# zhihu/ZhiLight

Hardware: AMD Instinct MI355X
Metric: decode tokens/s (Llama-3-8B GPTQ-Int4, TP=1 per GPU, batch 1, seq 1024) (higher is better)
Workload: dtype f16; 1 GPU; Llama-3-8B GPTQ-Int4 g128 TP=1 batch=1 decode seq=1024 (BASELINE configs[1]); layers=32, parallelism=dp1 (independent TP=1 replicas), global_batch=1, seq_len=1024, valid=True, kv_cache_dtype=fp16, w4_algo=mfma

## Files before the change

### include/zhilight_amd.h

```cpp
#ifndef ZHILIGHT_AMD_H
#define ZHILIGHT_AMD_H

#include <stddef.h>
#include <stdint.h>

#ifdef __cplusplus
extern "C" {
#endif

#define ZL_VERSION 100

enum { ZL_F16 = 0, ZL_BF16 = 1, ZL_F32 = 2  };

enum {
    ZL_OK = 0,
    ZL_EINVAL = -1,
    ZL_ESHAPE = -2,
    ZL_EDTYPE = -3,
    ZL_ELIMIT = -4
};

typedef void* zl_stream_t;

int zl_version(void);
// ... 36 lines not shown

int zl_moe_grouped_bm(int64_t pairs, int64_t num_experts);
int64_t zl_moe_grouped_tiles(int64_t pairs, int64_t num_experts, int64_t bm);
int zl_w4a16_gemm_grouped(const uint16_t* x, int64_t ldx, int64_t x_rows, const uint32_t* qw, const uint32_t* meta,
                          int64_t num_experts, int64_t expert_stride_qw, int64_t expert_stride_meta,
                          const int32_t* expert_loads, const int32_t* index, int64_t pairs, int in_div, int out_scatter,
                          uint16_t* y, int64_t y_rows, int64_t n, int64_t k, int64_t group_size, int epilogue, zl_stream_t s);
int zl_w4a16_gemm_pairs(const uint16_t* x, int64_t ldx, int64_t x_rows, const uint32_t* qw, const uint32_t* meta, int64_t num_experts,
                        int64_t expert_stride_qw, int64_t expert_stride_meta, const int32_t* expert_ids, int64_t pairs, int in_div,
                        uint16_t* y, int64_t n, int64_t k, int64_t group_size, int epilogue, zl_stream_t s);

enum {
    ZL_EPI_BIAS = 1, ZL_EPI_ADD_C = 2, ZL_EPI_RESIDUAL = 4, ZL_EPI_SILU_MUL = 8, ZL_EPI_SILU_MUL_F32 = 16
};

int zl_w4a16_gemm(const uint16_t* x, int64_t ldx,
                  const uint32_t* qw, const uint16_t* scales, const uint16_t* zeros,
                  const uint16_t* bias, const uint16_t* residual, uint16_t* y,
                  int64_t m, int64_t n, int64_t k, int64_t group_size, int sym,
                  const uint16_t* norm_weight, float norm_eps, int epilogue, zl_stream_t s);

int zl_w4m_layout(int64_t n, int64_t k, int64_t group_size, zl_w4_layout_t* out);
int zl_w4m_pack(const uint32_t* qweight_km, const uint8_t* qzeros_km, const uint16_t* scales_km,
                int64_t n, int64_t k, int64_t group_size, int row_interleave,
                uint32_t* qw, uint32_t* meta, zl_stream_t s);
int zl_w4m_unpack(const uint32_t* qw, const uint32_t* meta, int64_t n, int64_t k, int64_t group_size, int row_interleave,
                  uint32_t* qweight_km, uint8_t* qzeros_km, uint16_t* scales_km, zl_stream_t s);
int zl_w4a16_gemm_mfma(const uint16_t* x, int64_t ldx,
                       const uint32_t* qw, const uint32_t* meta,
                       const uint16_t* bias, const uint16_t* residual, uint16_t* y,
                       int64_t m, int64_t n, int64_t k, int64_t group_size,
                       const uint16_t* norm_weight, float norm_eps, int epilogue, zl_stream_t s);

#define ZL_SCRATCH_HEADER 65536
typedef struct {
    void* scratch;
    int64_t scratch_bytes;
    int phase_rounds, phase_ksplit, phase_ksplit_min_m, phase_min_m, phase_max_m, phase_small_off;
    int tiled_min_m, tiled_bm, tiled_splitk;
    int mfma_ks, mfma_rounds;
    int small_algo;
    int tiled_wide;
    int slab;
    int slab_min_m;
    int slab_nw, slab_gpw;
    int slab_r;
    int defer_norm;
    const float* row_ss;
    float* row_ss_out;
} zl_w4_opts_t;
int64_t zl_w4a16_scratch_bytes(int64_t m, int64_t n);
int zl_row_ss(const uint16_t* x, int64_t ldx, int64_t m, int64_t k, float* out, zl_stream_t s);
int zl_w4a16_emits_row_ss(int64_t m, int64_t n, int64_t k, int64_t group_size, int epilogue, const zl_w4_opts_t* opts);
int zl_w4a16_takes_row_ss(int64_t m, int64_t n, int64_t k, int64_t group_size, int rope, const zl_w4_opts_t* opts);
int zl_w4a16_gemm_mfma_ex(const uint16_t* x, int64_t ldx, const uint32_t* qw, const uint32_t* meta, const uint16_t* bias,
                          const uint16_t* residual, uint16_t* y, int64_t m, int64_t n, int64_t k, int64_t group_size,
                          const uint16_t* norm_weight, float norm_eps, int epilogue, const zl_w4_opts_t* opts, zl_stream_t s);
int zl_w4a16_gemm_tiled(const uint16_t* x, int64_t ldx, const uint32_t* qw, const uint32_t* meta,
                        const uint16_t* bias, const uint16_t* residual, uint16_t* y,
                        int64_t m, int64_t n, int64_t k, int64_t group_size, int epilogue, zl_stream_t s);
int zl_w4a16_gemm_tiled_ex(const uint16_t* x, int64_t ldx, const uint32_t* qw, const uint32_t* meta,
                           const uint16_t* bias, const uint16_t* residual, uint16_t* y, int64_t m, int64_t n, int64_t k,
                           int64_t group_size, int epilogue, const zl_w4_opts_t* opts, zl_stream_t s);


int zl_gemm_nt_small_m(const uint16_t* x, int64_t ldx, const uint16_t* w , const uint16_t* bias,
                       uint16_t* y, int64_t m, int64_t n, int64_t k, float alpha, int dtype,
                       const uint16_t* norm_weight, float norm_eps, zl_stream_t s);
int zl_gemm_nt(const uint16_t* x, int64_t ldx, const uint16_t* w , const uint16_t* bias, uint16_t* y,
               int64_t m, int64_t n, int64_t k, float alpha, int dtype, zl_stream_t s);
int64_t zl_dense_m_bytes(int64_t n, int64_t k);
int zl_dense_pack_m(const uint16_t* w, uint16_t* out, int64_t n, int64_t k, zl_stream_t s);
int zl_gemm_nt_packed(const uint16_t* x, int64_t ldx, const uint16_t* wp, const uint16_t* bias, uint16_t* y, int64_t m,
                      int64_t n, int64_t k, float alpha, int dtype, zl_stream_t s);
int zl_gemm_nt_f32(const uint16_t* x, int64_t ldx, const uint16_t* w , float* y, int64_t m, int64_t n, int64_t k, float alpha,
                   int dtype, zl_stream_t s);

int64_t zl_argmax_workspace_bytes(int64_t m, int64_t n);
int zl_gemm_nt_small_m_argmax(const uint16_t* x, int64_t ldx, const uint16_t* w , const uint16_t* bias,
                              uint16_t* y, int64_t m, int64_t n, int64_t k, float alpha, int dtype,
                              const uint16_t* norm_weight, float norm_eps, void* argmax_ws, zl_stream_t s);
int zl_greedy_advance(const void* argmax_ws, int64_t m, int64_t n, int32_t* tokens, int32_t* positions,
                      int32_t* placement, int32_t* valid_lens, int64_t* next_tokens, zl_stream_t s);

int64_t zl_lm_head_score_ws_bytes(int64_t m, int64_t n);
int zl_lm_head_score(const uint16_t* x, int64_t ldx, const uint16_t* w , const int32_t* labels, int32_t ignore_index,
                     int32_t col0, float* lse, float* label_logit, float* logprob, int32_t* greedy, float* greedy_logit,
                     void* workspace, int64_t m, int64_t n, int64_t k, int dtype, zl_stream_t s);
enum { ZL_SCORE_ORDER_AUTO = -1 };
int zl_lm_head_score_ex(const uint16_t* x, int64_t ldx, const uint16_t* w , const int32_t* labels, int32_t ignore_index,
                        int32_t col0, float* lse, float* label_logit, float* logprob, int32_t* greedy, float* greedy_logit,
                        void* workspace, int64_t m, int64_t n, int64_t k, int dtype, int order, zl_stream_t s);


int zl_fp8_calc_scale(const uint16_t* x, int64_t numel, float max_e4m3, float* scale, int dtype, zl_stream_t s);
int zl_fp8_cvt_half(const uint16_t* x, const float* scale, uint8_t* out, int64_t numel, int dtype, zl_stream_t s);
int zl_fp8_gemm_nt(const uint8_t* a , const uint8_t* b , const float* scale_a, const float* scale_b,
                   uint16_t* out , int64_t m, int64_t n, int64_t k, zl_stream_t s);

int zl_quant_group_32(const uint16_t* x, int8_t* q, uint16_t* scale, int64_t groups, int dtype, zl_stream_t s);
int zl_dequant_sum_quant_g32(const uint16_t* my , const int8_t* q_others ,
                             const uint16_t* scale_others , int8_t* q_sum, uint16_t* scale_sum,
                             int64_t groups, int world_size, int dtype, zl_stream_t s);
int zl_dequant_group_32(const int8_t* q, const uint16_t* scale, uint16_t* out, int64_t groups, int dtype, zl_stream_t s);

int zl_rmsnorm(const uint16_t* x, const uint16_t* weight, uint16_t* out, int64_t rows, int64_t dim,
               float eps, float scale, const uint16_t* x2, uint16_t* out_sum, int dtype, zl_stream_t s);

int zl_rope_cos_sin(const int32_t* pos, float* cosv, float* sinv, int64_t s_len, int64_t d, float base,
                    int neox, zl_stream_t s);
int zl_rope_cos_sin_llama3(const int32_t* pos, float* cosv, float* sinv, int64_t s_len, int64_t d, float base,
                           float factor, float low_freq_factor, float high_freq_factor,
                           float old_context_len, int neox, zl_stream_t s);
int zl_rope_cos_sin_dynamic(const int32_t* pos, const int32_t* seq_len, float* cosv, float* sinv, int64_t s_len, int64_t d,
                            float base, float factor, float max_position_embeddings, int neox, zl_stream_t s);
int zl_rope_cos_sin_yarn(const int32_t* pos, float* cosv, float* sinv, int64_t s_len, int64_t d, float base, float factor,
                         float low, float high, float mscale, int neox, zl_stream_t s);
int zl_head_norm(const uint16_t* x, const uint16_t* weight, uint16_t* out, int64_t rows, int64_t heads, int64_t d, int64_t ld_in,
                 int64_t ld_out, float eps, int mode, int dtype, zl_stream_t s);
int zl_rotary_embedding_qk(const int32_t* pos, const uint16_t* in, uint16_t* q, uint16_t* k, uint16_t* v,
                           int64_t s_len, int64_t h, int64_t hkv, int64_t d, float theta, int dtype,
                           zl_stream_t s);
int zl_rope_qk_cache(const float* cosv, const float* sinv, const uint16_t* in, uint16_t* q, uint16_t* k,
                     uint16_t* v, int64_t s_len, int64_t h, int64_t hkv, int64_t d, int neox, int dtype,
                     zl_stream_t s);
int zl_rope_rotate(const float* cosv, const float* sinv, const uint16_t* x, uint16_t* out, int64_t n, int64_t heads, int64_t d,
                   int64_t x_stride_n, int64_t x_stride_h, int64_t out_stride_n, int64_t out_stride_h, int neox, int dtype, zl_stream_t s);
int zl_mask_valid_lens(const int8_t* mask, const int32_t* buf_lens, int32_t* valid_lens, int64_t b, int64_t len_q, zl_stream_t s);

int zl_copy_to_rag_buffer2(const int32_t* placement, const int32_t* buf_lens, const uint16_t* k_src,
                           const uint16_t* v_src, uint16_t* const* k_bufs, uint16_t* const* v_bufs,
                           int64_t b, int64_t len_q, int64_t hkv, int64_t d, int bshd, zl_stream_t s);
int zl_copy_to_rag_buffer_bytes(const int32_t* placement, const int32_t* buf_lens, const void* k_src, const void* v_src, void* const* k_bufs,
                                void* const* v_bufs, int64_t b, int64_t len_q, int64_t hkv, int64_t row_bytes, int bshd, zl_stream_t s);
int zl_kv_blocks_copy(const int32_t* desc, int64_t n, void* const* k_bufs, void* const* v_bufs, const int32_t* buf_lens, void* pool,
                      int64_t layers, int64_t b, int64_t block, int64_t hkv, int64_t row_bytes, int bshd, int to_pool, zl_stream_t s);
int zl_kv_blocks_copy_ex(const int32_t* desc, int64_t n, void* const* k_bufs, void* const* v_bufs, const int32_t* buf_lens, void* pool,
                         int64_t layers, int64_t b, int64_t block, int64_t hkv, int64_t row_bytes, int bshd, int to_pool,
                         int64_t piece_bytes, zl_stream_t s);

int zl_rope_scatter_decode(const float* cosv, const float* sinv, const uint16_t* qkv ,
                           uint16_t* q , const int32_t* placement ,
                           const int32_t* buf_lens, uint16_t* const* k_bufs, uint16_t* const* v_bufs,
                           int64_t b, int64_t h, int64_t hkv, int64_t d, int neox, int bshd, int dtype,
                           zl_stream_t s);

int64_t zl_decode_attn_workspace_bytes(int64_t b, int64_t len_q, int64_t h, int64_t d, int64_t max_len_buf);
int zl_decode_attn(const uint16_t* q, const int32_t* buf_lens, const uint16_t* const* k_bufs,
                   const uint16_t* const* v_bufs, const int8_t* mask, const int32_t* valid_lens,
                   uint16_t* out, void* workspace, int64_t b, int64_t len_q, int64_t h, int64_t hkv,
                   int64_t d, float scale, int64_t max_len_buf, int bshd, int dtype, zl_stream_t s);
int zl_decode_attn_ex(const uint16_t* q, const int32_t* buf_lens, const uint16_t* const* k_bufs,
                      const uint16_t* const* v_bufs, const int8_t* mask, const int32_t* valid_lens,
                      uint16_t* out, void* workspace, int64_t b, int64_t len_q, int64_t h, int64_t hkv,
                      int64_t d, float scale, int64_t max_len_buf, int bshd, int dtype, int algo, zl_stream_t s);

int zl_decode_attn_causal(const uint16_t* q, const int32_t* buf_lens, const uint16_t* const* k_bufs,
                          const uint16_t* const* v_bufs, const int32_t* valid_lens, uint16_t* out, void* workspace,
                          int64_t b, int64_t len_q, int64_t h, int64_t hkv, int64_t d, float scale, int64_t max_len_buf,
                          int bshd, int dtype, zl_stream_t s);

int zl_decode_attn_fused(const float* cosv, const float* sinv, const uint16_t* qkv, const int32_t* placement,
                         const int32_t* buf_lens, const int32_t* valid_lens, uint16_t* const* k_bufs,
                         uint16_t* const* v_bufs, uint16_t* out, void* workspace, int64_t b, int64_t h,
                         int64_t hkv, int64_t d, float scale, int64_t max_len_buf, int neox, int bshd, int dtype,
                         zl_stream_t s);
// ... 320 lines not shown
```

### zhilight_amd/_lib.py

```python
import ctypes as C
import os

import torch

_HERE = os.path.dirname(os.path.abspath(__file__))
SO_PATH = os.environ.get("ZHILIGHT_AMD_SO") or os.path.join(_HERE, "libzhilight_amd.so")

SYMBOLS = [
    "zl_mla_decode_workspace_bytes", "zl_mla_decode_attn", "zl_mla_decode_attn_ex", "zl_mla_decode_attn_paged",
    "zl_moe_sum_experts", "zl_moe_sum_experts_arr", "zl_moe_route_shared_lb", "zl_moe_plus_for_sort", "zl_moe_calc_reverse_idx",
    "zl_moe_fill_m_indices",
    "zl_embedding_rope",
    "zl_fp8_per_token_cast", "zl_fp8_block_dequant", "zl_fp8_block_gemm_group", "zl_fp8_block_packed_bytes", "zl_fp8_block_pack", "zl_fp8_block_gemm_group_packed", "zl_moe_top_k_softmax", "zl_moe_group_topk",
    "zl_cast", "zl_copy_2d", "zl_index_select", "zl_argmax_advance", "zl_arange_i32", "zl_divide_i32", "zl_scatter_update_dim0", "zl_sort_pairs_i32", "zl_log_softmax_bias", "zl_softmax_rows", "zl_topk_rows", "zl_gather_logits", "zl_scatter_logits", "zl_repetition_penalty", "zl_spec_accept", "zl_lookup_draft", "zl_stop_advance", "zl_slots_admit", "zl_sample_advance", "zl_spec_sample_accept", "zl_sample_advance_ex", "zl_spec_sample_accept_ex", "zl_seen_mark", "zl_sample_advance_opts", "zl_spec_sample_accept_opts", "zl_sample_advance_fsm", "zl_spec_sample_accept_fsm", "zl_slots_admit_fsm", "zl_reduce_abs_max", "zl_binary_op", "zl_scale", "zl_act_inplace",
    "zl_count_nonfinite", "zl_perm_narrow_u16", "zl_perm_reverse_u16", "zl_permute_input_u16", "zl_gptq_permute_rows",
    "zl_version", "zl_status_string", "zl_device_cu_count",
    "zl_gptq_shuffle", "zl_gptq_increase_zero", "zl_gptq_q4_to_q8", "zl_transpose_2d", "zl_gptq_reconstruct",
    "zl_awq_un_shuffle", "zl_awq_shuffle",
    "zl_w4_layout", "zl_w4_pack", "zl_w4_dequant", "zl_w4a16_gemm",
    "zl_w4m_layout", "zl_w4m_pack", "zl_w4m_unpack", "zl_w4a16_gemm_mfma", "zl_w4a16_gemm_tiled", "zl_w4a16_scratch_bytes", "zl_w4a16_gemm_mfma_ex", "zl_w4a16_gemm_tiled_ex",
    "zl_gemm_nt_small_m", "zl_gemm_nt", "zl_gemm_nt_f32", "zl_argmax_workspace_bytes", "zl_gemm_nt_small_m_argmax", "zl_greedy_advance",
    "zl_lm_head_score_ws_bytes", "zl_lm_head_score", "zl_lm_head_score_ex",
    "zl_rmsnorm",
    "zl_w4a16_moe_up", "zl_w4a16_moe_down", "zl_moe_grouped_bm", "zl_moe_grouped_tiles", "zl_w4a16_gemm_grouped", "zl_w4a16_gemm_pairs", "zl_rope_cos_sin", "zl_rope_cos_sin_llama3", "zl_rope_cos_sin_dynamic", "zl_rope_cos_sin_yarn", "zl_head_norm", "zl_rotary_embedding_qk", "zl_rope_qk_cache", "zl_rope_rotate", "zl_mask_valid_lens",
    "zl_copy_to_rag_buffer2", "zl_copy_to_rag_buffer_bytes", "zl_kv_blocks_copy", "zl_kv_blocks_copy_ex", "zl_rope_scatter_decode", "zl_w4a16_qkv_rope_scatter", "zl_w4a16_qkv_rope_scatter_ex", "zl_decode_attn_splits_h", "zl_decode_attn_splits_h_mask", "zl_decode_attn_combine_h", "zl_w4a16_gemm_attn_merge_h", "zl_w4a16_gemm_attn_merge_h_ex",
    "zl_quant_group_32", "zl_dequant_sum_quant_g32", "zl_dequant_group_32",
    "zl_fp8_calc_scale", "zl_fp8_cvt_half", "zl_fp8_gemm_nt",
    "zl_decode_attn_workspace_bytes", "zl_decode_attn", "zl_decode_attn_ex", "zl_decode_attn_causal", "zl_decode_attn_fused",
    "zl_decode_attn_split_len", "zl_decode_attn_splits", "zl_w4a16_gemm_attn_merge",
    "zl_decode_attn_la_split_len", "zl_decode_attn_la_workspace_bytes", "zl_decode_attn_la",
    "zl_quant_calc_scale_zp", "zl_dequant_group", "zl_quant_copy_to_rag_buffer", "zl_rope_quant_scatter_decode", "zl_decode_attn_quant", "zl_decode_attn_quant_ex",
    "zl_prefill_attn", "zl_prefill_attn_ex", "zl_prefill_attn_varlen", "zl_prefill_attn_varlen_q8",
    "zl_element_add_scale", "zl_gate_mul", "zl_gate_fuse", "zl_dense_m_bytes", "zl_dense_pack_m", "zl_gemm_nt_packed", "zl_row_ss", "zl_w4a16_emits_row_ss", "zl_w4a16_takes_row_ss", "zl_permute_input", "zl_embedding",
    "zl_w8m_bytes", "zl_w8m_pack", "zl_w8a8_gemm_phase", "zl_w8a8_gemm_phase_ex", "zl_w8a8_qkv_rope_scatter",
    "zl_quant_calc_scale", "zl_rmsnorm_quant", "zl_int8_gemm_nt", "zl_quant_scale_back",
    "zl_quant_back_act_mul", "zl_quant_scale_back3", "zl_quant_back_element_add_scale", "zl_quant_back_transpose",
    "zl_quant_back_copy_to_buffer",
    "zl_w4a8_weight_to_int8", "zl_quant_scale_back_f32",
    "zl_awq_dequantize", "zl_awq_gemm_workspace_bytes", "zl_awq_gemm",
]


EXPERIMENTAL_SYMBOLS = ["zl_w4a16_attn_out_gate_up", "zl_engine_epoch_advance",
                        "zl_w4a16_planes_bytes", "zl_w4a16_planes", "zl_w4a16_gemm_planes", "zl_w4a16_qkv_rope_scatter_planes"]
experimental = False


class W4Opts(C.Structure):
    _fields_ = [("scratch", C.c_void_p), ("scratch_bytes", C.c_int64)] + [(n, C.c_int) for n in (
        "phase_rounds", "phase_ksplit", "phase_ksplit_min_m", "phase_min_m", "phase_max_m", "phase_small_off",
        "tiled_min_m", "tiled_bm", "tiled_splitk", "mfma_ks", "mfma_rounds", "small_algo", "tiled_wide",
        "slab", "slab_min_m", "slab_nw", "slab_gpw", "slab_r", "defer_norm")] + [("row_ss", C.c_void_p), ("row_ss_out", C.c_void_p)]


class W4Layout(C.Structure):
    _fields_ = [(n, C.c_int64) for n in
                ("n", "k", "group_size", "np", "kp", "q", "c", "qw_bytes", "scales_bytes", "zeros_bytes")]


_lib = None


def lib():
    global _lib
    if _lib is None:
        if not os.path.exists(SO_PATH):
            raise ImportError(
                f"{SO_PATH} not found: build it with `python -m zhilight_amd.build` "
                "(hipcc --offload-arch=gfx950). zhilight_amd has no CPU/PyTorch fallback.")
        l = C.CDLL(SO_PATH)
        for name in SYMBOLS:
            getattr(l, name)
        l.zl_status_string.restype = C.c_char_p
        l.zl_decode_attn_workspace_bytes.restype = C.c_int64
        l.zl_decode_attn_split_len.restype = C.c_int64
        l.zl_decode_attn_la_split_len.restype = C.c_int64
        l.zl_decode_attn_la_workspace_bytes.restype = C.c_int64
        l.zl_argmax_workspace_bytes.restype = C.c_int64
        l.zl_lm_head_score_ws_bytes.restype = C.c_int64
        l.zl_w8m_bytes.restype = C.c_int64
        l.zl_dense_m_bytes.restype = C.c_int64
        l.zl_fp8_block_packed_bytes.restype = C.c_int64
        l.zl_mla_decode_workspace_bytes.restype = C.c_int64
        l.zl_w4a16_scratch_bytes.restype = C.c_int64
        l.zl_moe_grouped_tiles.restype = C.c_int64
        global experimental
        experimental = all(hasattr(l, name) for name in EXPERIMENTAL_SYMBOLS)
        if experimental:
            l.zl_w4a16_planes_bytes.restype = C.c_int64
        l.zl_awq_gemm_workspace_bytes.restype = C.c_int64
        l.zl_sample_advance.restype = C.c_int
        l.zl_sample_advance.argtypes = [C.c_void_p, C.c_int] + [C.c_int64] * 3 + [C.c_void_p] * 14
        l.zl_spec_sample_accept.restype = C.c_int
        l.zl_spec_sample_accept.argtypes = [C.c_void_p, C.c_int] + [C.c_int64] * 4 + [C.c_void_p] * 17
        l.zl_sample_advance_ex.restype = C.c_int
        l.zl_sample_advance_ex.argtypes = [C.c_void_p, C.c_int] + [C.c_int64] * 3 + [C.c_void_p] * 16 + [C.c_int64, C.c_void_p]
        l.zl_spec_sample_accept_ex.restype = C.c_int
        l.zl_spec_sample_accept_ex.argtypes = [C.c_void_p, C.c_int] + [C.c_int64] * 4 + [C.c_void_p] * 19 + [C.c_int64, C.c_void_p]
        opts = [C.c_void_p] * 3 + [C.c_int64, C.c_void_p, C.c_int64, C.c_int, C.c_void_p, C.c_void_p]
        l.zl_sample_advance_opts.restype = C.c_int
        l.zl_sample_advance_opts.argtypes = [C.c_void_p, C.c_int] + [C.c_int64] * 3 + [C.c_void_p] * 16 + [C.c_int64] + opts + [C.c_void_p]
        l.zl_spec_sample_accept_opts.restype = C.c_int
        l.zl_spec_sample_accept_opts.argtypes = [C.c_void_p, C.c_int] + [C.c_int64] * 4 + [C.c_void_p] * 19 + [C.c_int64] + opts + [C.c_void_p]
        fsm = [C.c_void_p, C.c_int64] + [C.c_void_p] * 4 + [C.c_int64] * 2 + [C.c_void_p]
# ... 56 lines not shown
```

### zhilight_amd/csrc/dense_gemv.hip

```cpp
#include "zl_common.h"
#include "zl_stage.h"

namespace {

constexpr int kRing = 8;

struct DenseParams {
    const uint16_t* x;
    int64_t ldx;
    const uint16_t* w;
    const uint16_t* bias;
    uint16_t* y;
    const uint16_t* norm_w;
    float norm_eps, alpha;
    int m, n, k, kp;
    int loads_per_row;
    int rows_per_wave;
    float2* argmax_ws;
    int total_waves;
};

typedef _Float16 hv2 __attribute__((ext_vector_type(2)));

template <int DT>
__device__ __forceinline__ float dot8(uint4 a, uint4 b, float acc) {
    const uint32_t au[4] = {a.x, a.y, a.z, a.w}, bu[4] = {b.x, b.y, b.z, b.w};
#pragma unroll
    for (int e = 0; e < 4; ++e) {
        if constexpr (DT == ZL_F16) {
            acc = __builtin_amdgcn_fdot2(__builtin_bit_cast(hv2, au[e]), __builtin_bit_cast(hv2, bu[e]), acc, false);
        } else {
            acc = __builtin_fmaf(__builtin_bit_cast(float, au[e] << 16), __builtin_bit_cast(float, bu[e] << 16), acc);
            acc = __builtin_fmaf(__builtin_bit_cast(float, au[e] & 0xffff0000u),
                                 __builtin_bit_cast(float, bu[e] & 0xffff0000u), acc);
        }
    }
    return acc;
}

template <int DT, int MT>
__global__ __launch_bounds__(256) void k_dense_gemv(const DenseParams p) {
    extern __shared__ __attribute__((aligned(16))) unsigned char smem[];
    uint16_t* xs = reinterpret_cast<uint16_t*>(smem);
    float* red = reinterpret_cast<float*>(smem + (size_t)MT * p.kp * 2);

    const int lane = threadIdx.x & 63;
    const int wave = __builtin_amdgcn_readfirstlane(threadIdx.x >> 6);
    const int m0 = blockIdx.y * MT;
    const int L = p.loads_per_row;
    const int gw = blockIdx.x * 4 + wave;
    const int row0 = gw * p.rows_per_wave;
    int nrows = p.n - row0;
    nrows = nrows < 0 ? 0 : (nrows > p.rows_per_wave ? p.rows_per_wave : nrows);
    const int total = nrows * L;

    uint4 wq[kRing];
    int iss_row = row0, iss_l = 0;
    auto issue = [&](int slot) {
        const int col = iss_l * 512 + lane * 8;
        uint4 v = make_uint4(0, 0, 0, 0);
        if (col < p.k) v = zl_load_nt(reinterpret_cast<const uint4*>(p.w + (size_t)iss_row * p.k + col));
        wq[slot] = v;
        if (++iss_l == L) {
            iss_l = 0;
            ++iss_row;
        }
    };
#pragma unroll
    for (int s = 0; s < kRing; ++s)
        if (s < total) issue(s);

    zl_stage_rows<DT, MT, 256>(p.x, p.ldx, m0, p.m, p.k, p.kp, p.norm_w, p.norm_eps, xs, red);
    __syncthreads();

    float acc[MT];
    float best_v[MT];
    int best_i[MT];
#pragma unroll
    for (int m = 0; m < MT; ++m) {
        acc[m] = 0.f;
        best_v[m] = -INFINITY;
        best_i[m] = 0x7fffffff;
    }
    int cl = 0, crow = row0;
    auto consume = [&](int slot) {
#pragma unroll
        for (int m = 0; m < MT; ++m) {
            uint4 xa = *reinterpret_cast<const uint4*>(xs + (size_t)m * p.kp + cl * 512 + lane * 8);
            acc[m] = dot8<DT>(wq[slot], xa, acc[m]);
        }
        if (++cl == L) {
            cl = 0;
#pragma unroll
            for (int m = 0; m < MT; ++m) {
                float v = zl_wave_sum(acc[m]);
                acc[m] = 0.f;
                if (lane == 0 && (m0 + m) < p.m) {
                    float b = p.bias ? ZT<DT>::to_f32(p.bias[crow]) : 0.f;
                    const uint16_t y16 = ZT<DT>::from_f32(p.alpha * v + b);
                    p.y[(size_t)(m0 + m) * p.n + crow] = y16;
                    const float yv = ZT<DT>::to_f32(y16);
                    if (yv > best_v[m] || best_i[m] == 0x7fffffff || (yv != yv && best_v[m] == best_v[m])) {
                        best_v[m] = yv;
                        best_i[m] = crow;
                    }
                }
            }
            ++crow;
        }
    };
#pragma unroll 1
    for (int it = 0; it < total; it += kRing) {
#pragma unroll
        for (int s = 0; s < kRing; ++s) {
            if (it + s < total) {
                consume(s);
                if (it + s + kRing < total) issue(s);
            }
        }
    }
    if (p.argmax_ws && lane == 0) {
#pragma unroll
        for (int m = 0; m < MT; ++m)
            if ((m0 + m) < p.m)
                p.argmax_ws[(size_t)(m0 + m) * p.total_waves + gw] = make_float2(best_v[m], __int_as_float(best_i[m]));
    }
}

__device__ __forceinline__ bool greedy_beats(float v, int i, float bv, int bi) {
    if (i == 0x7fffffff) return false;
    if (bi == 0x7fffffff) return true;
    if (v != v) return bv == bv || i < bi;
    return v > bv || (v == bv && i < bi);
}

__global__ __launch_bounds__(256) void k_greedy_advance(const float2* ws, int total_waves, int32_t* tokens,
                                                        int32_t* positions, int32_t* placement, int32_t* valid_lens,
                                                        int64_t* next_out) {
    __shared__ float sv[256];
    __shared__ int si[256];
    const int b = blockIdx.x;
    float bv = -INFINITY;
    int bi = 0x7fffffff;
    for (int w0 = threadIdx.x; w0 < total_waves; w0 += 4 * 256) {
        float2 c[4];
#pragma unroll
        for (int u = 0; u < 4; ++u) {
            const int w = w0 + u * 256;
            c[u] = w < total_waves ? ws[(size_t)b * total_waves + w] : make_float2(0.f, __int_as_float(0x7fffffff));
        }
#pragma unroll
        for (int u = 0; u < 4; ++u) {
            const int ci = __float_as_int(c[u].y);
            if (greedy_beats(c[u].x, ci, bv, bi)) {
                bv = c[u].x;
                bi = ci;
            }
        }
    }
    sv[threadIdx.x] = bv;
    si[threadIdx.x] = bi;
    __syncthreads();
    for (int off = 128; off > 0; off >>= 1) {
        if ((int)threadIdx.x < off) {
            const float ov = sv[threadIdx.x + off];
            const int oi = si[threadIdx.x + off];
            if (greedy_beats(ov, oi, sv[threadIdx.x], si[threadIdx.x])) {
                sv[threadIdx.x] = ov;
                si[threadIdx.x] = oi;
            }
        }
        __syncthreads();
    }
    if (threadIdx.x == 0) {
        const int tok = si[0] == 0x7fffffff ? 0 : si[0];
        if (tokens) tokens[b] = tok;
        if (next_out) next_out[b] = tok;
        if (positions) positions[b] += 1;
        if (placement) placement[b] += 1;
        if (valid_lens) valid_lens[b] += 1;
    }
}

template <int DT, int MT>
int launch(const DenseParams& p, int gx, int gy, hipStream_t st) {
    size_t lds = (size_t)MT * p.kp * 2 + 64;
    if (lds > 160 * 1024) return ZL_ELIMIT;
    if (lds > 64 * 1024) {
        hipError_t e = hipFuncSetAttribute(reinterpret_cast<const void*>(&k_dense_gemv<DT, MT>),
                                           hipFuncAttributeMaxDynamicSharedMemorySize, (int)lds);
        if (e != hipSuccess) return (int)e;
    }
    hipLaunchKernelGGL((k_dense_gemv<DT, MT>), dim3(gx, gy), dim3(256), lds, st, p);
    return zl_launch_status();
}

template <int DT>
__global__ __launch_bounds__(64) void k_gemm_nt_f32(const uint16_t* __restrict__ x, int64_t ldx, const uint16_t* __restrict__ w, float* __restrict__ y,
                                                    int n, int k, float alpha) {
    const int col = blockIdx.x, row = blockIdx.y, lane = threadIdx.x;
    const uint16_t* xr = x + (int64_t)row * ldx;
    const uint16_t* wr = w + (int64_t)col * k;
    float acc = 0.f;
    for (int i = lane * 8; i + 8 <= k; i += 64 * 8) {
        const uint4 a = *reinterpret_cast<const uint4*>(xr + i), b = *reinterpret_cast<const uint4*>(wr + i);
        const uint32_t au[4] = {a.x, a.y, a.z, a.w}, bu[4] = {b.x, b.y, b.z, b.w};
#pragma unroll
        for (int e = 0; e < 4; ++e) {
            acc = __builtin_fmaf(ZT<DT>::to_f32((uint16_t)(au[e] & 0xffffu)), ZT<DT>::to_f32((uint16_t)(bu[e] & 0xffffu)), acc);
            acc = __builtin_fmaf(ZT<DT>::to_f32((uint16_t)(au[e] >> 16)), ZT<DT>::to_f32((uint16_t)(bu[e] >> 16)), acc);
        }
    }
    acc = zl_wave_sum(acc);
    if (lane == 0) y[(int64_t)row * n + col] = alpha * acc;
}

}

static int dense_waves(int64_t n, int* rows_per_wave, int* gx) {
    int cus = zl_device_cu_count();
    if (cus <= 0) cus = 256;
    const int waves = cus * 8;
    *rows_per_wave = (int)((n + waves - 1) / waves);
    *gx = (int)(((n + *rows_per_wave - 1) / *rows_per_wave + 3) / 4);
    return *gx * 4;
}

extern "C" int64_t zl_argmax_workspace_bytes(int64_t m, int64_t n) {
    if (m <= 0 || n <= 0) return ZL_EINVAL;
    int rpw, gx;
    return m * (int64_t)dense_waves(n, &rpw, &gx) * 8;
}

static int gemm_nt_small_m_impl(const uint16_t* x, int64_t ldx, const uint16_t* w, const uint16_t* bias, uint16_t* y,
                                int64_t m, int64_t n, int64_t k, float alpha, int dtype, const uint16_t* norm_weight,
                                float norm_eps, void* argmax_ws, zl_stream_t s) {
    ZL_CHECK_ARG(x && w && y && m > 0 && n > 0 && k > 0, ZL_EINVAL);
    ZL_CHECK_ARG(k % 8 == 0 && ldx % 8 == 0 && ldx >= k, ZL_ESHAPE);
    ZL_CHECK_ARG(dtype == ZL_F16 || dtype == ZL_BF16, ZL_EDTYPE);
    DenseParams p;
    p.x = x; p.ldx = ldx; p.w = w; p.bias = bias; p.y = y;
    p.norm_w = norm_weight; p.norm_eps = norm_eps; p.alpha = alpha;
    p.m = (int)m; p.n = (int)n; p.k = (int)k;
    p.kp = (int)((k + 511) / 512 * 512);
    p.loads_per_row = p.kp / 512;
    int mt = m >= 4 ? 4 : (int)m;
    while (mt > 1 && (size_t)mt * p.kp * 2 + 64 > 64 * 1024) --mt;
    if (mt == 3) mt = 2;
    const int gy = (int)((m + mt - 1) / mt);
    int gx;
    p.total_waves = dense_waves(n, &p.rows_per_wave, &gx);
    p.argmax_ws = reinterpret_cast<float2*>(argmax_ws);
    hipStream_t hs = (hipStream_t)s;
#define ZL_DISPATCH(DT)                                      \
    switch (mt) {                                            \
        case 1: return launch<DT, 1>(p, gx, gy, hs);         \
        case 2: return launch<DT, 2>(p, gx, gy, hs);         \
        default: return launch<DT, 4>(p, gx, gy, hs);        \
    }
    if (dtype == ZL_F16) { ZL_DISPATCH(ZL_F16) }
    ZL_DISPATCH(ZL_BF16)
#undef ZL_DISPATCH
}

extern "C" int zl_gemm_nt_small_m(const uint16_t* x, int64_t ldx, const uint16_t* w, const uint16_t* bias, uint16_t* y,
                                  int64_t m, int64_t n, int64_t k, float alpha, int dtype,
                                  const uint16_t* norm_weight, float norm_eps, zl_stream_t s) {
    return gemm_nt_small_m_impl(x, ldx, w, bias, y, m, n, k, alpha, dtype, norm_weight, norm_eps, nullptr, s);
}

extern "C" int zl_gemm_nt_small_m_argmax(const uint16_t* x, int64_t ldx, const uint16_t* w, const uint16_t* bias,
                                         uint16_t* y, int64_t m, int64_t n, int64_t k, float alpha, int dtype,
                                         const uint16_t* norm_weight, float norm_eps, void* argmax_ws, zl_stream_t s) {
    ZL_CHECK_ARG(argmax_ws, ZL_EINVAL);
    return gemm_nt_small_m_impl(x, ldx, w, bias, y, m, n, k, alpha, dtype, norm_weight, norm_eps, argmax_ws, s);
}

extern "C" int zl_gemm_nt_f32(const uint16_t* x, int64_t ldx, const uint16_t* w, float* y, int64_t m, int64_t n, int64_t k, float alpha, int dtype,
                              zl_stream_t s) {
    ZL_CHECK_ARG(x && w && y && m > 0 && n > 0 && k > 0, ZL_EINVAL);
    ZL_CHECK_ARG(k % 8 == 0 && ldx >= k && ldx % 8 == 0 && ((uintptr_t)x & 15) == 0 && ((uintptr_t)w & 15) == 0 && m <= 65535 && n < ((int64_t)1 << 31), ZL_ESHAPE);
    ZL_CHECK_ARG(dtype == ZL_F16 || dtype == ZL_BF16, ZL_EDTYPE);
    const dim3 grid((unsigned)n, (unsigned)m);
    if (dtype == ZL_F16) hipLaunchKernelGGL(k_gemm_nt_f32<ZL_F16>, grid, dim3(64), 0, (hipStream_t)s, x, ldx, w, y, (int)n, (int)k, alpha);
    else hipLaunchKernelGGL(k_gemm_nt_f32<ZL_BF16>, grid, dim3(64), 0, (hipStream_t)s, x, ldx, w, y, (int)n, (int)k, alpha);
    return zl_launch_status();
}

extern "C" int zl_greedy_advance(const void* argmax_ws, int64_t m, int64_t n, int32_t* tokens, int32_t* positions,
                                 int32_t* placement, int32_t* valid_lens, int64_t* next_tokens, zl_stream_t s) {
    ZL_CHECK_ARG(argmax_ws && m > 0 && n > 0, ZL_EINVAL);
    int rpw, gx;
    const int tw = dense_waves(n, &rpw, &gx);
    hipLaunchKernelGGL(k_greedy_advance, dim3((unsigned)m), dim3(256), 0, (hipStream_t)s,
                       reinterpret_cast<const float2*>(argmax_ws), tw, tokens, positions, placement, valid_lens, next_tokens);
    return zl_launch_status();
}
```

### zhilight_amd/csrc/misc_ops.hip

```cpp
#include <mutex>
#include "zl_common.h"

namespace {

template <int DT>
__global__ __launch_bounds__(256) void k_rmsnorm(const uint16_t* __restrict__ x, const uint16_t* __restrict__ w,
                                                 uint16_t* __restrict__ out, int dim, float eps, float scale,
                                                 const uint16_t* __restrict__ x2, uint16_t* __restrict__ out_sum) {
    extern __shared__ __attribute__((aligned(16))) unsigned char smem[];
    float* vbuf = reinterpret_cast<float*>(smem);
    float* red = vbuf + dim;
    const size_t off = (size_t)blockIdx.x * dim;
    float ss = 0.f;
    for (int i = threadIdx.x * 8; i < dim; i += 256 * 8) {
        uint4 a = *reinterpret_cast<const uint4*>(x + off + i);
        uint4 b = make_uint4(0, 0, 0, 0);
        if (x2) b = *reinterpret_cast<const uint4*>(x2 + off + i);
        const uint32_t au[4] = {a.x, a.y, a.z, a.w}, bu[4] = {b.x, b.y, b.z, b.w};
        uint32_t su[4];
#pragma unroll
        for (int e = 0; e < 4; ++e) {
            float v0 = ZT<DT>::to_f32((uint16_t)(au[e] & 0xffff)), v1 = ZT<DT>::to_f32((uint16_t)(au[e] >> 16));
            if (x2) {
                v0 += ZT<DT>::to_f32((uint16_t)(bu[e] & 0xffff));
                v1 += ZT<DT>::to_f32((uint16_t)(bu[e] >> 16));
                su[e] = (uint32_t)ZT<DT>::from_f32(v0) | ((uint32_t)ZT<DT>::from_f32(v1) << 16);
            }
            vbuf[i + 2 * e] = v0;
            vbuf[i + 2 * e + 1] = v1;
            ss = __builtin_fmaf(v0, v0, ss);
            ss = __builtin_fmaf(v1, v1, ss);
        }
        if (x2 && out_sum) *reinterpret_cast<uint4*>(out_sum + off + i) = make_uint4(su[0], su[1], su[2], su[3]);
    }
    ss = zl_block_sum(ss, red);
    const float rs = zl_rsqrt_rn(ss / (float)dim + eps);
    for (int i = threadIdx.x * 8; i < dim; i += 256 * 8) {
        uint4 wv = *reinterpret_cast<const uint4*>(w + i);
        const uint32_t wu[4] = {wv.x, wv.y, wv.z, wv.w};
        uint32_t o[4];
#pragma unroll
        for (int e = 0; e < 4; ++e) {
            float a = vbuf[i + 2 * e] * rs * ZT<DT>::to_f32((uint16_t)(wu[e] & 0xffff)) / scale;
            float b = vbuf[i + 2 * e + 1] * rs * ZT<DT>::to_f32((uint16_t)(wu[e] >> 16)) / scale;
            o[e] = (uint32_t)ZT<DT>::from_f32(a) | ((uint32_t)ZT<DT>::from_f32(b) << 16);
        }
        *reinterpret_cast<uint4*>(out + off + i) = make_uint4(o[0], o[1], o[2], o[3]);
    }
}

__device__ __forceinline__ int half_dim_index(int col, int half_dim, int neox) {
    return neox ? (col < half_dim ? col : col - half_dim) : col / 2;
}

__device__ __forceinline__ void rope_cos_sin_row(int row, const int32_t* __restrict__ pos, float* __restrict__ cosv, float* __restrict__ sinv,
                                                 int d, float base, int neox, int llama3, float factor, float low_ff, float high_ff,
                                                 float old_ctx) {
    const int col = threadIdx.x;
    if (col >= d) return;
    const int i = half_dim_index(col, d / 2, neox);
    float inv_freq = (float)pow((double)base, (double)(-(float)(i * 2) / (float)d));
    if (llama3) {
        const float low_wl = old_ctx / low_ff, high_wl = old_ctx / high_ff;
        const float pi = 3.141592653589793f;
        const float wavelen = 2.f * pi / inv_freq;
        if (wavelen < high_wl) {
        } else if (wavelen > low_wl) {
            inv_freq = inv_freq / factor;
        } else {
            const float smooth = (old_ctx / wavelen - low_ff) / (high_ff - low_ff);
            inv_freq = __builtin_fmaf(smooth, inv_freq, (1.f - smooth) * inv_freq / factor);
        }
    }
    const float freq = (float)pos[row] * inv_freq;
    cosv[(size_t)row * d + col] = cosf(freq);
    sinv[(size_t)row * d + col] = sinf(freq);
}
__global__ void k_rope_cos_sin(const int32_t* __restrict__ pos, float* __restrict__ cosv, float* __restrict__ sinv,
                               int d, float base, int neox, int llama3, float factor, float low_ff, float high_ff,
                               float old_ctx) {
    rope_cos_sin_row(blockIdx.x, pos, cosv, sinv, d, base, neox, llama3, factor, low_ff, high_ff, old_ctx);
}

__global__ void k_rope_cos_sin_scaled(const int32_t* __restrict__ pos, const int32_t* __restrict__ seq_len,
                                      float* __restrict__ cosv, float* __restrict__ sinv, int d, float base, int neox, int type,
                                      float factor, float p1, float p2, float p3) {
    const int col = threadIdx.x;
    if (col >= d) return;
    const int i = half_dim_index(col, d / 2, neox);
    const int t = blockIdx.x;
    float freq, scale = 1.f;
    if (type == 2) {
        float theta = base;
        const int len = seq_len ? seq_len[t] : pos[t];
        if ((float)len > p1) theta *= (float)pow((double)((factor * (float)len / p1) - (factor - 1.f)), (double)(float)(d / (d - 2)));
        freq = (float)pos[t] * (float)pow((double)theta, (double)(-(float)(i * 2) / (float)d));
    } else {
        const float pos_freq = (float)pow((double)base, (double)((float)(i * 2) / (float)d));
        const float extrap = 1.0f / pos_freq, interp = 1.0f / (factor * pos_freq);
        const float fi = (float)i;
        const float ramp = fi <= p1 ? 0.f : (fi >= p2 ? 1.f : (fi - p1) / (p2 - p1));
        freq = (float)pos[t] * __builtin_fmaf(interp, ramp, extrap * (1.f - ramp));
        scale = p3;
    }
    cosv[(size_t)t * d + col] = cosf(freq) * scale;
    sinv[(size_t)t * d + col] = sinf(freq) * scale;
}

template <int DT>
__global__ void k_head_norm(const uint16_t* __restrict__ x, const uint16_t* __restrict__ w, uint16_t* __restrict__ out, int d,
                            int64_t ld_in, int64_t ld_out, float eps, int mode) {
    __shared__ float red[16];
    const int col = threadIdx.x, head = blockIdx.y;
    const int64_t row = blockIdx.x;
    float v = col < d ? ZT<DT>::to_f32(x[row * ld_in + (int64_t)head * d + col]) : 0.f;
    if (mode == 1) {
        const float mean = zl_block_sum(v, red) / (float)d;
        v = col < d ? v - mean : 0.f;
    }
    const float var = zl_block_sum(v * v, red) / (float)d;
    const float r = zl_rsqrt_rn(var + eps);
    if (col < d) {
        const float wv = ZT<DT>::to_f32(w[(mode == 1 ? (int64_t)head * d : 0) + col]);
        out[row * ld_out + (int64_t)head * d + col] = ZT<DT>::from_f32(v * r * wv);
    }
}

__device__ __forceinline__ float rope_val(float a, float b, float c, float s, bool minus) {
    return minus ? __builtin_fmaf(-b, s, a * c) : __builtin_fmaf(b, s, a * c);
}

template <int DT, int MODE>
__global__ void k_rope_qk(const int32_t* __restrict__ pos, const float* __restrict__ cosv,
                          const float* __restrict__ sinv, const uint16_t* __restrict__ in, uint16_t* __restrict__ q,
                          uint16_t* __restrict__ k, uint16_t* __restrict__ v, int h, int hkv, int d, float theta,
                          int neox) {
    const int t = blockIdx.x, head = blockIdx.y, col = threadIdx.x, all = h + 2 * hkv, half = d / 2;
    if (col >= d) return;
    const uint16_t* src = in + ((size_t)t * all + head) * d;
    if (head >= h + hkv) {
        v[((size_t)t * hkv + (head - h - hkv)) * d + col] = src[col];
        return;
    }
    float c, s;
    if (MODE == 0) {
        const int i = col < half ? col : col - half;
        const float freq = (float)pos[t] * (float)pow((double)theta, (double)(-(float)(i * 2) / (float)d));
        c = cosf(freq);
        s = sinf(freq);
    } else {
        c = cosv[(size_t)t * d + col];
        s = sinv[(size_t)t * d + col];
    }
    const float a = ZT<DT>::to_f32(src[col]);
    float r;
    if (MODE == 0 || neox)
        r = col < half ? rope_val(a, ZT<DT>::to_f32(src[col + half]), c, s, true)
                       : rope_val(a, ZT<DT>::to_f32(src[col - half]), c, s, false);
    else
        r = (col & 1) == 0 ? rope_val(a, ZT<DT>::to_f32(src[col + 1]), c, s, true)
// ... 119 lines not shown
        *reinterpret_cast<uint32_t*>(v_bufs[b] + dof + i) = *reinterpret_cast<const uint32_t*>(v_src + so + i);
    }
}

template <int DT>
__global__ void k_rope_scatter_decode(const float* __restrict__ cosv, const float* __restrict__ sinv,
                                      const uint16_t* __restrict__ qkv, uint16_t* __restrict__ q,
                                      const int32_t* __restrict__ placement, const int32_t* __restrict__ buf_lens,
                                      uint16_t* const* __restrict__ k_bufs, uint16_t* const* __restrict__ v_bufs, int h,
                                      int hkv, int d, int neox, int bshd) {
    const int t = blockIdx.x, head = blockIdx.y, col = threadIdx.x, all = h + 2 * hkv, half = d / 2;
    if (col >= d) return;
    const uint16_t* src = qkv + ((size_t)t * all + head) * d;
    const int64_t len_buf = buf_lens[t];
    const int p = placement[t] < len_buf ? placement[t] : -1;
    if (head >= h + hkv) {
        if (p < 0) return;
        const int hk = head - h - hkv;
        const size_t dof = bshd ? ((size_t)p * hkv + hk) * d : ((size_t)hk * len_buf + p) * d;
        v_bufs[t][dof + col] = src[col];
        return;
    }
    const float c = cosv[(size_t)t * d + col], s = sinv[(size_t)t * d + col];
    const float a = ZT<DT>::to_f32(src[col]);
    float r;
    if (neox)
        r = col < half ? rope_val(a, ZT<DT>::to_f32(src[col + half]), c, s, true)
                       : rope_val(a, ZT<DT>::to_f32(src[col - half]), c, s, false);
    else
        r = (col & 1) == 0 ? rope_val(a, ZT<DT>::to_f32(src[col + 1]), c, s, true)
                           : rope_val(a, ZT<DT>::to_f32(src[col - 1]), c, s, false);
    const uint16_t o = ZT<DT>::from_f32(r);
    if (head < h) {
        q[((size_t)t * h + head) * d + col] = o;
    } else if (p >= 0) {
        const int hk = head - h;
        const size_t dof = bshd ? ((size_t)p * hkv + hk) * d : ((size_t)hk * len_buf + p) * d;
        k_bufs[t][dof + col] = o;
    }
}

template <int DT>
__device__ __forceinline__ uint16_t t_add(uint16_t a, uint16_t b) {
    return ZT<DT>::from_f32(ZT<DT>::to_f32(a) + ZT<DT>::to_f32(b));
}
template <int DT>
__device__ __forceinline__ uint16_t t_mul(uint16_t a, uint16_t b) {
    return ZT<DT>::from_f32(ZT<DT>::to_f32(a) * ZT<DT>::to_f32(b));
}

template <int DT>
__global__ void k_add_scale(const uint16_t* __restrict__ a, const uint16_t* __restrict__ b, uint16_t* __restrict__ c,
                            int64_t n, uint16_t scale_t, int scale_residual) {
    for (int64_t i = blockIdx.x * (int64_t)blockDim.x + threadIdx.x; i < n; i += (int64_t)gridDim.x * blockDim.x)
        c[i] = scale_residual ? t_mul<DT>(t_add<DT>(a[i], b[i]), scale_t) : t_add<DT>(a[i], t_mul<DT>(b[i], scale_t));
}

template <int DT>
__global__ void k_gate_mul(const uint16_t* __restrict__ g, const uint16_t* __restrict__ u, uint16_t* __restrict__ out,
                           int64_t n, int act) {
    for (int64_t i = blockIdx.x * (int64_t)blockDim.x + threadIdx.x; i < n; i += (int64_t)gridDim.x * blockDim.x) {
        const float x = ZT<DT>::to_f32(g[i]);
        float a;
        if (act == 0) a = x / (1.0f + expf(-x));
        else a = 0.5f * x * (1.0f + tanhf(0.7978845608028654f * x * (1.0f + 0.044715f * x * x)));
        out[i] = ZT<DT>::from_f32(a * ZT<DT>::to_f32(u[i]));
    }
}

template <int DT>
__global__ void k_gate_fuse(const uint16_t* __restrict__ in, uint16_t* __restrict__ out, int64_t rows, int64_t ff, int act) {
    const int64_t n = rows * ff;
    for (int64_t i = blockIdx.x * (int64_t)blockDim.x + threadIdx.x; i < n; i += (int64_t)gridDim.x * blockDim.x) {
        const int64_t r = i / ff, j = i - r * ff;
        const float x = ZT<DT>::to_f32(in[r * 2 * ff + j]);
        float a;
        if (act == 0) a = x / (1.0f + expf(-x));
        else a = 0.5f * x * (1.0f + tanhf(0.7978845608028654f * x * (1.0f + 0.044715f * x * x)));
        out[i] = ZT<DT>::from_f32(a * ZT<DT>::to_f32(in[r * 2 * ff + ff + j]));
    }
}

template <int DT>
__device__ __forceinline__ void embedding_row(int row, const int32_t* __restrict__ ids, const uint16_t* __restrict__ w,
                                              uint16_t* __restrict__ out, int dim, int begin, int end, float scale) {
    int id = ids[row];
    const bool in_range = id >= begin && id < end;
    id -= begin;
    const uint16_t* src = w + (size_t)(in_range ? id : 0) * dim;
    uint16_t* dst = out + (size_t)row * dim;
    if ((dim & 7) == 0 && ((((uintptr_t)w) | ((uintptr_t)out)) & 15) == 0) {
        const int chunks = dim >> 3;
        for (int c0 = threadIdx.x; c0 < chunks; c0 += 2 * blockDim.x) {
            const int c1 = c0 + blockDim.x;
            uint4 v0 = *reinterpret_cast<const uint4*>(src + (size_t)c0 * 8), v1 = make_uint4(0, 0, 0, 0);
            if (c1 < chunks) v1 = *reinterpret_cast<const uint4*>(src + (size_t)c1 * 8);
            auto conv = [&](uint32_t u) {
                const uint16_t lo = in_range ? ZT<DT>::from_f32(ZT<DT>::to_f32((uint16_t)(u & 0xffffu)) * scale) : ZT<DT>::from_f32(0.f);
                const uint16_t hi = in_range ? ZT<DT>::from_f32(ZT<DT>::to_f32((uint16_t)(u >> 16)) * scale) : ZT<DT>::from_f32(0.f);
                return (uint32_t)lo | ((uint32_t)hi << 16);
            };
            *reinterpret_cast<uint4*>(dst + (size_t)c0 * 8) = make_uint4(conv(v0.x), conv(v0.y), conv(v0.z), conv(v0.w));
            if (c1 < chunks) *reinterpret_cast<uint4*>(dst + (size_t)c1 * 8) = make_uint4(conv(v1.x), conv(v1.y), conv(v1.z), conv(v1.w));
        }
        return;
    }
    for (int i = threadIdx.x; i < dim; i += blockDim.x)
        dst[i] = in_range ? ZT<DT>::from_f32(ZT<DT>::to_f32(src[i]) * scale) : ZT<DT>::from_f32(0.f);
}
template <int DT>
__global__ void k_embedding(const int32_t* __restrict__ ids, const uint16_t* __restrict__ w, uint16_t* __restrict__ out,
                            int dim, int begin, int end, float scale) {
    embedding_row<DT>(blockIdx.x, ids, w, out, dim, begin, end, scale);
}
template <int DT>
__global__ __launch_bounds__(256) void k_embedding_rope(const int32_t* __restrict__ ids, const uint16_t* __restrict__ w, uint16_t* __restrict__ out,
                                                        int dim, int begin, int end, float scale, int s_len, const int32_t* __restrict__ pos,
                                                        float* __restrict__ cosv, float* __restrict__ sinv, int d, float base, int neox,
                                                        int llama3, float factor, float low_ff, float high_ff, float old_ctx) {
    if ((int)blockIdx.x < s_len) embedding_row<DT>(blockIdx.x, ids, w, out, dim, begin, end, scale);
    else rope_cos_sin_row(blockIdx.x - s_len, pos, cosv, sinv, d, base, neox, llama3, factor, low_ff, high_ff, old_ctx);
}

inline int grid_1d(int64_t n, int threads) {
    int64_t g = (n + threads - 1) / threads;
    return (int)(g > 4096 ? 4096 : (g < 1 ? 1 : g));
}

}

#define ZL_DT_SWITCH(dtype, EXPR_F16, EXPR_BF16) \
    if ((dtype) == ZL_F16) { EXPR_F16; } else if ((dtype) == ZL_BF16) { EXPR_BF16; } else return ZL_EDTYPE;

extern "C" {

int zl_version(void) { return ZL_VERSION; }

const char* zl_status_string(int st) {
    switch (st) {
        case ZL_OK: return "ok";
        case ZL_EINVAL: return "invalid argument (null pointer or non-positive size)";
        case ZL_ESHAPE: return "shape/alignment not supported by this kernel";
        case ZL_EDTYPE: return "dtype not supported on this path";
        case ZL_ELIMIT: return "exceeds a hardware limit (LDS / grid)";
        default: return st > 0 ? hipGetErrorString((hipError_t)st) : "unknown status";
    }
}

int zl_device_cu_count(void) {
    int dev = 0;
    hipError_t e = hipGetDevice(&dev);
    if (e != hipSuccess) return -(int)e;
    static int cache[64] = {0};
    if (dev >= 0 && dev < 64 && cache[dev] > 0) return cache[dev];
    int cus = 0;
    e = hipDeviceGetAttribute(&cus, hipDeviceAttributeMultiprocessorCount, dev);
    if (e != hipSuccess) return -(int)e;
    if (dev >= 0 && dev < 64) cache[dev] = cus;
    return cus;
}

int zl_rmsnorm(const uint16_t* x, const uint16_t* weight, uint16_t* out, int64_t rows, int64_t dim, float eps,
               float scale, const uint16_t* x2, uint16_t* out_sum, int dtype, zl_stream_t s) {
    ZL_CHECK_ARG(x && weight && out && rows > 0 && dim > 0, ZL_EINVAL);
    ZL_CHECK_ARG(dim % 8 == 0, ZL_ESHAPE);
    size_t lds = (size_t)dim * 4 + 64;
    ZL_CHECK_ARG(lds <= 64 * 1024, ZL_ELIMIT);
    ZL_DT_SWITCH(dtype,
        hipLaunchKernelGGL(k_rmsnorm<ZL_F16>, dim3((unsigned)rows), dim3(256), lds, (hipStream_t)s, x, weight, out, (int)dim, eps, scale, x2, out_sum),
        hipLaunchKernelGGL(k_rmsnorm<ZL_BF16>, dim3((unsigned)rows), dim3(256), lds, (hipStream_t)s, x, weight, out, (int)dim, eps, scale, x2, out_sum))
    return zl_launch_status();
}

int zl_rope_cos_sin(const int32_t* pos, float* cosv, float* sinv, int64_t s_len, int64_t d, float base, int neox,
                    zl_stream_t s) {
    ZL_CHECK_ARG(pos && cosv && sinv && s_len > 0 && d > 0, ZL_EINVAL);
    ZL_CHECK_ARG(d <= 1024 && d % 2 == 0, ZL_ESHAPE);
    hipLaunchKernelGGL(k_rope_cos_sin, dim3((unsigned)s_len), dim3((unsigned)d), 0, (hipStream_t)s, pos, cosv, sinv,
                       (int)d, base, neox, 0, 1.f, 1.f, 1.f, 1.f);
    return zl_launch_status();
}

int zl_rope_cos_sin_llama3(const int32_t* pos, float* cosv, float* sinv, int64_t s_len, int64_t d, float base,
                           float factor, float low_freq_factor, float high_freq_factor, float old_context_len,
                           int neox, zl_stream_t s) {
    ZL_CHECK_ARG(pos && cosv && sinv && s_len > 0 && d > 0, ZL_EINVAL);
    ZL_CHECK_ARG(d <= 1024 && d % 2 == 0, ZL_ESHAPE);
    hipLaunchKernelGGL(k_rope_cos_sin, dim3((unsigned)s_len), dim3((unsigned)d), 0, (hipStream_t)s, pos, cosv, sinv,
                       (int)d, base, neox, 1, factor, low_freq_factor, high_freq_factor, old_context_len);
    return zl_launch_status();
}

int zl_rope_cos_sin_dynamic(const int32_t* pos, const int32_t* seq_len, float* cosv, float* sinv, int64_t s_len, int64_t d, float base,
// ... 178 lines not shown
```

### zhilight_amd/csrc/w4_i8p.hip

```cpp
#include "zl_common.h"
#include "w4_i8p_common.h"

namespace {

constexpr int kT = 512, kW = 8;
#ifndef ZL_I8P_RING
#define ZL_I8P_RING 8
#endif
#ifndef ZL_I8P_EARLY
#define ZL_I8P_EARLY 0
#endif

#ifdef ZL_I8P_PROBE
__device__ unsigned long long* zl_probe_i8 = nullptr;
#define ZL_IPROBE_INIT()                                                                               \
    unsigned long long* pp_ = nullptr;                                                                 \
    if (zl_probe_i8 && (threadIdx.x & 63) == 0 && blockIdx.x < 2048)                                   \
        pp_ = zl_probe_i8 + ((size_t)blockIdx.x * kW + (threadIdx.x >> 6)) * 8;
#define ZL_IPROBE(slot)                                                                                \
    do {                                                                                               \
        if (pp_) pp_[slot] = wall_clock64();                                                           \
    } while (0)
#else
#define ZL_IPROBE_INIT() do {} while (0)
#define ZL_IPROBE(slot) do {} while (0)
#endif

template <int R, bool LONGK, bool ROPE, bool NORM, bool MERGE = false>
__global__ __launch_bounds__(kT, 2) void k_w4a16_i8p(const I8Params p) {
    static_assert(!ROPE || R == 2, "fused rotary: a tile and its partner tile");
    static_assert(!MERGE || (!LONGK && !ROPE && !NORM), "split merge: one column block, plain prologue");
    constexpr int XD = R >= ZL_I8P_RING ? 1 : (ZL_I8P_RING / R > 0 ? ZL_I8P_RING / R : 1);
    constexpr int D = R * XD;
    constexpr int NS = LONGK ? 8 : 4;
    constexpr int NR = LONGK ? 2 : 4;
    extern __shared__ __attribute__((aligned(16))) unsigned char smem[];
    ZL_IPROBE_INIT();
    ZL_IPROBE(0);
    const int lane = threadIdx.x & 63;
    const int wave = __builtin_amdgcn_readfirstlane(threadIdx.x >> 6);
    const int M = p.m, K = p.k, groups = p.groups;
    const int rec = 64 * M;
    const int Gw = (groups + kW - 1) / kW;
    unsigned char* planes = smem + (size_t)wave * Gw * 8 * rec;
    float* consts = reinterpret_cast<float*>(smem + (size_t)kW * Gw * 8 * rec) + (size_t)wave * Gw * 16;
    float* red = reinterpret_cast<float*>(smem + (size_t)kW * Gw * 8 * rec) + (size_t)kW * Gw * 16;
    float* scratch = red + R * kW * 64;

    const int tile0 = ROPE ? (blockIdx.x / p.pair_stride) * 2 * p.pair_stride + blockIdx.x % p.pair_stride : blockIdx.x * R;
    const int tile_stride = ROPE ? p.pair_stride : 1;
    const int my_groups = wave < groups ? (groups - wave + kW - 1) / kW : 0;

    constexpr int E = ZL_I8P_EARLY < D ? ZL_I8P_EARLY : D;
    uint4 wq[D];
    uint32_t mt[D];
    const __amdgpu_buffer_rsrc_t rq = __builtin_amdgcn_make_buffer_rsrc(const_cast<uint4*>(p.qw), 0, p.qw_bytes, 0x00020000);
    const __amdgpu_buffer_rsrc_t rm = __builtin_amdgcn_make_buffer_rsrc(const_cast<uint32_t*>(p.meta), 0, p.meta_bytes, 0x00020000);
    const __amdgpu_buffer_rsrc_t rnull = __builtin_amdgcn_make_buffer_rsrc(const_cast<uint4*>(p.qw), 0, 0, 0x00020000);
    const uint32_t q_off = (uint32_t)lane * 16u, m_off = (uint32_t)(lane & 15) * 4u;
    auto issue = [&](int slot, int gi, int r) {
        const int g = wave + kW * gi;
        const bool ok = g < groups;
        const uint32_t it = (uint32_t)(tile0 + r * tile_stride) * (uint32_t)groups + (uint32_t)g;
        wq[slot] = __builtin_bit_cast(uint4, __builtin_amdgcn_raw_buffer_load_b128(ok ? rq : rnull, q_off, it * 1024u, 2 ));
        mt[slot] = __builtin_amdgcn_raw_buffer_load_b32(ok ? rm : rnull, m_off, it * 64u, 2);
    };
    auto issue_early = [&]() {
        if constexpr (E > 0) {
            __builtin_amdgcn_sched_barrier(0);
#pragma unroll
            for (int q = 0; q < E; ++q) issue(q, q / R, q % R);
            __builtin_amdgcn_sched_barrier(0);
        }
    };

    uint4 xr[NS], nw[LONGK ? 4 : 1];
    const int lgi = lane >> 4, uo = lane & 15;
#pragma unroll
    for (int c = 0; c < (LONGK ? 4 : 1); ++c) {
        nw[c] = make_uint4(0, 0, 0, 0);
        const int g = wave + kW * (4 * c + lgi);
        if (NORM && 4 * c < Gw) nw[c] = *reinterpret_cast<const uint4*>(p.norm_w + (g < groups ? g * 128 + uo * 8 : 0));
    }
#pragma unroll
    for (int s = 0; s < NS; ++s) {
        const int row = LONGK ? (s & 1) : s, c = LONGK ? (s >> 1) : 0;
        const int g = wave + kW * (4 * c + lgi);
        xr[s] = make_uint4(0, 0, 0, 0);
        if constexpr (MERGE) {
            if (row < M) {
                constexpr int kS = 16;
                const int head = g < groups ? g : 0;
                const uint32_t n_rec = (uint32_t)M * (uint32_t)groups * (uint32_t)p.mg_max_splits;
                const __amdgpu_buffer_rsrc_t rpart = __builtin_amdgcn_make_buffer_rsrc(const_cast<uint16_t*>(p.mg_part), 0, n_rec * 256u, 0x00020000);
                const __amdgpu_buffer_rsrc_t rstat = __builtin_amdgcn_make_buffer_rsrc(const_cast<float*>(p.mg_stat), 0, n_rec * 8u, 0x00020000);
                const uint32_t rec0 = ((uint32_t)row * (uint32_t)groups + (uint32_t)head) * (uint32_t)p.mg_max_splits;
                const uint32_t po = rec0 * 256u + (uint32_t)uo * 16u, so = rec0 * 8u;
                uint4 pv[kS];
                float2 st[kS];
#pragma unroll
                for (int u = 0; u < kS; ++u) {
                    const uint32_t uc = u < p.mg_max_splits ? (uint32_t)u : 0u;
                    pv[u] = __builtin_bit_cast(uint4, __builtin_amdgcn_raw_buffer_load_b128(rpart, po, uc * 256u, 0));
                    st[u] = __builtin_bit_cast(float2, __builtin_amdgcn_raw_buffer_load_b64(rstat, so, uc * 8u, 0));
                }
                if (s == 0) issue_early();
                const int elen = min(p.buf_lens[row], p.mg_valid_lens[row]);
                const int ns = min((elen + p.mg_split_len - 1) / p.mg_split_len, kS);
                float mn = -1e20f;
#pragma unroll
                for (int u = 0; u < kS; ++u) mn = fmaxf(mn, u < ns ? st[u].x : -1e20f);
                float a[8] = {0.f, 0.f, 0.f, 0.f, 0.f, 0.f, 0.f, 0.f}, z = 0.f;
#pragma unroll
                for (int u = 0; u < kS; ++u) {
                    if (u < ns) {
                        const float f = st[u].y * __expf(st[u].x - mn);
                        const uint32_t w4[4] = {pv[u].x, pv[u].y, pv[u].z, pv[u].w};
#pragma unroll
                        for (int e = 0; e < 4; ++e) {
                            const h16x2 hh = __builtin_bit_cast(h16x2, w4[e]);
                            a[2 * e] = __builtin_fmaf((float)hh.x, f, a[2 * e]);
                            a[2 * e + 1] = __builtin_fmaf((float)hh.y, f, a[2 * e + 1]);
                        }
                        z += f;
                    }
                }
                const float zi = 1.0f / (z + 1e-20f);
                uint32_t o[4];
#pragma unroll
                for (int e = 0; e < 4; ++e) {
                    h16x2 hh;
                    hh.x = zl_f32_to_f16(a[2 * e] * zi);
                    hh.y = zl_f32_to_f16(a[2 * e + 1] * zi);
                    o[e] = __builtin_bit_cast(uint32_t, hh);
                }
                if (g < groups) xr[s] = make_uint4(o[0], o[1], o[2], o[3]);
            }
        } else
        if (row < M && 4 * c < Gw) {
            xr[s] = *reinterpret_cast<const uint4*>(p.x + (g < groups ? (size_t)row * p.ldx + g * 128 + uo * 8 : 0));
            if (g >= groups) xr[s] = make_uint4(0, 0, 0, 0);
        }
    }
    ZlRopeOperands rp;
    if constexpr (ROPE) {
        if ((int)threadIdx.x < 16 * M) rp = zl_rope_prefetch(p, threadIdx.x >> 4, tile0 * 16 + (threadIdx.x & 15));
    }
    const bool silu = (p.epi & (ZL_EPI_SILU_MUL | ZL_EPI_SILU_MUL_F32)) != 0;
    float ep_b0 = 0.f, ep_b1 = 0.f, ep_res = 0.f, ep_prev = 0.f;
    int ep_r = 0, ep_m = 0, ep_nl = 0, ep_col = -1;
    if constexpr (!ROPE) {
        const int per_tile = (silu ? 8 : 16) * M;
        if ((int)threadIdx.x < R * per_tile) {
            ep_r = threadIdx.x / per_tile;
            const int rem = threadIdx.x % per_tile, tile = tile0 + ep_r;
            if (!silu) {
                ep_m = rem >> 4; ep_nl = rem & 15;
                const int row = tile * 16 + ep_nl;
                if (tile < p.tiles && row < p.n) {
                    ep_col = row;
                    if ((p.epi & ZL_EPI_BIAS) && p.bias) ep_b0 = (float)__builtin_bit_cast(_Float16, p.bias[row]);
                    if (p.epi & ZL_EPI_ADD_C) ep_prev = (float)__builtin_bit_cast(_Float16, p.y[(size_t)ep_m * p.ld_out + row]);
                    if (p.epi & ZL_EPI_RESIDUAL) ep_res = (float)__builtin_bit_cast(_Float16, p.residual[(size_t)ep_m * p.ld_out + row]);
                }
            } else {
                ep_m = rem >> 3; ep_nl = rem & 7;
                const int pr = tile * 8 + ep_nl;
                if (tile < p.tiles && 2 * pr + 1 < p.n) {
                    ep_col = pr;
                    if ((p.epi & ZL_EPI_BIAS) && p.bias) {
                        ep_b0 = (float)__builtin_bit_cast(_Float16, p.bias[2 * pr]);
                        ep_b1 = (float)__builtin_bit_cast(_Float16, p.bias[2 * pr + 1]);
                    }
                }
            }
        }
    }
    if constexpr (!MERGE) issue_early();
    __builtin_amdgcn_sched_barrier(0);
    static_assert(2 * E < 16, "vmcnt immediate");
    __builtin_amdgcn_s_waitcnt(0x0F70 | (2 * E));
    __builtin_amdgcn_sched_barrier(0);
    ZL_IPROBE(1);

#define ZL_ISSUE_RANGE(LO, HI)                                     \
    {                                                              \
        __builtin_amdgcn_sched_barrier(0);                         \
        _Pragma("unroll") for (int q = ((LO) > E ? (LO) : E); q < (HI); ++q) issue(q, q / R, q % R); \
        __builtin_amdgcn_sched_barrier(0);                         \
    }
    constexpr int Q0 = NORM ? D / 2 : 0, NP = LONGK ? 8 : 4;
#define ZL_QLO(pos) (Q0 + ((D - Q0) * (pos) + NP - 1) / NP)

    float rs[NR];
#pragma unroll
    for (int r = 0; r < NR; ++r) rs[r] = 1.f;
    if constexpr (NORM) {
        float part[NR];
#pragma unroll
// ... 102 lines not shown
    asm volatile("s_waitcnt lgkmcnt(0)" ::: "memory");
    __builtin_amdgcn_wave_barrier();
    ZL_IPROBE(3);

    const int kq = lane >> 4, row16 = lane & 15;
    const int aslot = (row16 < 4 * M && (row16 & 3) != 3) ? row16 : 3;
    const unsigned char* a_base = planes + (size_t)kq * rec + aslot * 16;
    const int crow = min(kq, M - 1);
    float acc[R];
#pragma unroll
    for (int r = 0; r < R; ++r) acc[r] = 0.f;
    const uint32_t m4 = __builtin_amdgcn_readfirstlane(0x0f0f0f0fu);
    const v4i zero4 = (v4i){0, 0, 0, 0};

    for (int gi0 = 0; gi0 < my_groups; gi0 += XD) {
#pragma unroll
        for (int j = 0; j < XD; ++j) {
            const int gi = gi0 + j;
            if (j > 0 && gi >= my_groups) break;
            const v4i a0 = *reinterpret_cast<const v4i*>(a_base + (size_t)(gi * 2 + 0) * 4 * rec);
            const v4i a1 = *reinterpret_cast<const v4i*>(a_base + (size_t)(gi * 2 + 1) * 4 * rec);
            const float4 cst = *reinterpret_cast<const float4*>(consts + ((size_t)gi * 4 + crow) * 4);
#pragma unroll
            for (int r = 0; r < R; ++r) {
                const int slot = j * R + r;
                const uint4 w = wq[slot];
                const uint32_t mw = mt[slot];
                v4i b0, b1;
                b0[0] = (int)(w.x & m4); b0[1] = (int)((w.x >> 4) & m4); b0[2] = (int)(w.y & m4); b0[3] = (int)((w.y >> 4) & m4);
                b1[0] = (int)(w.z & m4); b1[1] = (int)((w.z >> 4) & m4); b1[2] = (int)(w.w & m4); b1[3] = (int)((w.w >> 4) & m4);
                v4i d = __builtin_amdgcn_mfma_i32_16x16x64_i8(a0, b0, zero4, 0, 0, 0);
                d = __builtin_amdgcn_mfma_i32_16x16x64_i8(a1, b1, d, 0, 0, 0);
                issue(slot, gi + XD, r);
                const h16x2 sm = __builtin_bit_cast(h16x2, mw);
                const float f12 = (float)((d[1] << 8) + d[2]), f0 = (float)d[0];
                float t = __builtin_fmaf((float)sm.y, cst.z, cst.w);
                t = __builtin_fmaf(f12, cst.x, t);
                t = __builtin_fmaf(f0, cst.y, t);
                asm volatile("" : "+v"(t) : "v"(b0), "v"(b1), "v"(a0), "v"(a1));
                acc[r] = __builtin_fmaf((float)sm.x, t, acc[r]);
#ifdef ZL_I8P_PROBE
                if (gi == 0 && r == 0) ZL_IPROBE(4);
#endif
            }
        }
    }

    ZL_IPROBE(5);
#pragma unroll
    for (int r = 0; r < R; ++r) red[(r * kW + wave) * 64 + lane] = acc[r];
    __syncthreads();
    ZL_IPROBE(6);
    auto total_of = [&](int r, int n_local, int m) {
        float v = 0.f;
#pragma unroll
        for (int w = 0; w < kW; ++w) v += red[(r * kW + w) * 64 + m * 16 + n_local];
        return v;
    };
    if constexpr (ROPE) {
        if ((int)threadIdx.x < 16 * M) {
            const int m = threadIdx.x >> 4, n_local = threadIdx.x & 15;
            zl_rope_store_f16(p, rp, m, tile0 * 16 + n_local, total_of(0, n_local, m), total_of(1, n_local, m));
        }
        ZL_IPROBE(7);
        return;
    }
    if (ep_col >= 0) {
        if (!silu) {
            const _Float16 y16 = zl_w4m_finish(total_of(ep_r, ep_nl, ep_m), ep_b0, ep_prev, ep_res, p.epi);
            p.y[(size_t)ep_m * p.ld_out + ep_col] = __builtin_bit_cast(uint16_t, y16);
        } else {
            const float g = total_of(ep_r, 2 * ep_nl, ep_m) + ep_b0, u = total_of(ep_r, 2 * ep_nl + 1, ep_m) + ep_b1;
            p.y[(size_t)ep_m * p.ld_out + ep_col] = __builtin_bit_cast(uint16_t, zl_f32_to_f16(zl_w4m_finish_gated(g, u, p.epi)));
        }
    }
    ZL_IPROBE(7);
}

static size_t i8p_lds_bytes(int groups, int m, int r) {
    const size_t gw = (groups + kW - 1) / kW;
    return kW * gw * 8 * 64 * (size_t)m + kW * gw * 64 + (size_t)r * kW * 64 * 4 + 4 * kW * 4;
}

template <int R, bool LONGK, bool ROPE, bool NORM, bool MERGE = false>
int launch_i8p_n(const I8Params& p, int grid, hipStream_t hs) {
    const size_t lds = i8p_lds_bytes(p.groups, p.m, R);
    if (lds > 160 * 1024) return ZL_ELIMIT;
    if (lds > 64 * 1024) {
        hipError_t e = hipFuncSetAttribute(reinterpret_cast<const void*>(&k_w4a16_i8p<R, LONGK, ROPE, NORM, MERGE>),
                                           hipFuncAttributeMaxDynamicSharedMemorySize, (int)lds);
        if (e != hipSuccess) return ZL_ELIMIT;
    }
    hipLaunchKernelGGL((k_w4a16_i8p<R, LONGK, ROPE, NORM, MERGE>), dim3(grid), dim3(kT), lds, hs, p);
    return zl_launch_status();
}
template <int R, bool ROPE>
int launch_i8p(const I8Params& p, int grid, hipStream_t hs) {
    const bool lk = p.groups > 4 * kW;
    if (p.norm_w) return lk ? launch_i8p_n<R, true, ROPE, true>(p, grid, hs) : launch_i8p_n<R, false, ROPE, true>(p, grid, hs);
    return lk ? launch_i8p_n<R, true, ROPE, false>(p, grid, hs) : launch_i8p_n<R, false, ROPE, false>(p, grid, hs);
}

}

#ifdef ZL_I8P_PROBE
extern "C" int zl_debug_set_probe_i8p(void* p) { return (int)hipMemcpyToSymbol(HIP_SYMBOL(zl_probe_i8), &p, sizeof(p)); }
#endif

bool zl_w4a16_i8p_covers(int64_t m, int64_t k) {
    if (m < 1 || m > 4 || k < 128 || k % 128 != 0 || k > 16384 || (k > 4096 && m > 2)) return false;
    return i8p_lds_bytes((int)(k / 128), (int)m, 8) <= 160 * 1024;
}

int zl_w4a16_gemm_i8p(const W4Problem& pb, int rounds_override, hipStream_t hs) {
    if (!zl_w4a16_i8p_covers(pb.m, pb.k)) return ZL_ESHAPE;
    const I8Params p = i8_params(pb);
    const int cus = zl_cu_count();
    int r = (pb.tiles + cus - 1) / cus;
    if (r > 8) r = 8;
    if (rounds_override > 0 && rounds_override <= 8) r = rounds_override;
    const int grid = (pb.tiles + r - 1) / r;
#define ZL_I8(RR) case RR: return launch_i8p<RR, false>(p, grid, hs);
    switch (r) { ZL_I8(1) ZL_I8(2) ZL_I8(3) ZL_I8(4) ZL_I8(5) ZL_I8(6) ZL_I8(7) ZL_I8(8) }
#undef ZL_I8
    return ZL_EINVAL;
}

int zl_w4a16_gemm_i8p_rope(const W4Problem& pb, const W4Rope& rp, hipStream_t hs) {
    if (!zl_w4a16_i8p_covers(pb.m, pb.k) || !zl_w4m_rope_shape_ok(pb, rp)) return ZL_ESHAPE;
    I8Params p = i8_params(pb);
    i8_fill_rope(p, rp);
    return launch_i8p<2, true>(p, pb.tiles / 2, hs);
}

int zl_w4a16_gemm_i8p_merge(const W4Problem& pb, const W4Merge& mg, hipStream_t hs) {
    if (pb.m < 1 || pb.m > 4 || pb.k > 4096 || pb.k % 128 != 0 || mg.max_splits < 1 || mg.max_splits > 16 || mg.split_len < 1) return ZL_ESHAPE;
    if (pb.epilogue & (ZL_EPI_SILU_MUL | ZL_EPI_SILU_MUL_F32)) return ZL_ESHAPE;
    I8Params p = i8_params(pb);
    i8_fill_merge(p, mg);
    const int cus = zl_cu_count();
    int r = (pb.tiles + cus - 1) / cus;
    if (r > 8) r = 8;
    const int grid = (pb.tiles + r - 1) / r;
#define ZL_I8M(RR) case RR: return launch_i8p_n<RR, false, false, false, true>(p, grid, hs);
    switch (r) { ZL_I8M(1) ZL_I8M(2) ZL_I8M(3) ZL_I8M(4) ZL_I8M(5) ZL_I8M(6) ZL_I8M(7) ZL_I8M(8) }
#undef ZL_I8M
    return ZL_EINVAL;
}
```

### zhilight_amd/llama.py

```python
import collections
import math
import os
import re
from dataclasses import dataclass, field
from typing import Dict, List, Optional

import numpy as np
import torch

from . import ops
from . import parallel


@dataclass
class ModelConfig:
    num_layers: int = 32
    dim_model: int = 4096
    num_heads: int = 32
    dim_head: int = 128
    dim_ff: int = 14336
    vocab_size: int = 128256
    num_kv_heads: int = 8
    eps: float = 1e-5
    rope_theta: float = 500000.0
# ... 682 lines not shown
            raise ops.ZLError(f"{prefix}: shared experts are not supported")
        super().load_state_dict(sd, prefix, device, ff=False)

        def lin(sub, din, dout):
            l = Int4GPTQ(prefix + "." + sub, din, dout, q)
            l.load_state_dict(sd, prefix + "." + sub, device)
            return l
        router = sd[prefix + ".ff.router.weight"]
        if tuple(router.shape) != (c.moe_num_experts, c.dim_model):
            raise ops.ZLError(f"{prefix}: router weight shape {tuple(router.shape)} != {(c.moe_num_experts, c.dim_model)}")
        self.router = _dev_t(router, device).to(torch.float16).contiguous()
        e, ff = c.moe_num_experts, c.moe_intermediate_size
        stack = ops.W4MMoEWeight if self.route == "grouped" else ops.W4MoEWeight
        up_parts, down_parts = ([], [], []), ([], [], [])
        for i in range(e):
            g, u = lin(f"ff.experts.{i}.w_in", c.dim_model, ff), lin(f"ff.experts.{i}.w_gated", c.dim_model, ff)
            for j in range(3):
                up_parts[j].append(torch.cat([g.km[j], u.km[j]]).contiguous())
            d = lin(f"ff.experts.{i}.w_out", ff, c.dim_model)
            for j in range(3):
                down_parts[j].append(d.km[j])
        self.w_up = stack.from_k_major(*up_parts, q.group_size, row_interleave=True)
        self.w_down = stack.from_k_major(*down_parts, q.group_size)

    def init_random(self, device, gen):
        raise ops.ZLError("MoE layers: use LLaMA.init_synthetic (the real load path)")

    def linears(self):
        return [self.qkv, self.attn_out]

    def weight_bytes(self):
        return sum(l.weight.nbytes() for l in self.linears()) + self.w_up.nbytes() + self.w_down.nbytes() + self.router.numel() * 2

    def moe(self, xn):
        c = self.cfg
        t, e, k = xn.shape[0], c.moe_num_experts, c.moe_top_k
        logits = ops.gemm_nt_f32(xn, self.router)
        loads = torch.zeros(e + 1, dtype=torch.int32, device=xn.device)
        weights, ids = ops.moe_top_k_softmax(logits, k, norm_topk_prob=c.norm_topk_prob, worker_load=loads[e:], expert_load=loads[:e])
        self.last_route = (ids, weights)
        if self.route == "fused":
            return ops.moe_down(ops.moe_up(xn, self.w_up, ids), self.w_down, ids, weights)
        p = t * k
        pair = ops.arange_i32(p, xn.device)
        if t <= self.m_thres:
            act = ops.moe_gemm_pairs(xn, self.w_up, ids, in_div=k, epilogue=ops.EPI_SILU_MUL)
            return ops.moe_sum_experts(ops.moe_gemm_pairs(act, self.w_down, ids), pair, weights)
        _, order = ops.sort_pairs_i32(ids.reshape(-1), pair, max_key=e)
        act = ops.moe_gemm_grouped(xn, self.w_up, loads[:e], order, p, in_div=k, epilogue=ops.EPI_SILU_MUL)
        down = ops.moe_gemm_grouped(act, self.w_down, loads[:e], order, p, out_scatter=True)
        return ops.moe_sum_experts(down, pair, weights)

    def ff_add(self, hidden, eps, act_buf=None):
        ops.element_add_scale(hidden, self.moe(ops.rmsnorm(hidden, self.ln_ff, eps)), 1.0, True, out=hidden)

    def ff_in(self, hidden, eps, out=None, normed=None):
        raise ops.ZLError("MoE layers have no gate|up projection of their own (ff_add runs the experts)")


ScoreResult = collections.namedtuple("ScoreResult", "logprobs lse greedy greedy_logit cu sums matches logits")


@dataclass
class DynBatchContext:
    tokens: torch.Tensor
    positions: torch.Tensor
    placement: torch.Tensor
    buf_lens: torch.Tensor
    valid_lens: torch.Tensor
    k_addrs: torch.Tensor
    v_addrs: torch.Tensor
    max_len_buf: int
    kv: List[torch.Tensor] = field(default_factory=list)
    kv_quant: bool = False
    ks_addrs: Optional[torch.Tensor] = None
    vs_addrs: Optional[torch.Tensor] = None
    kv_scales: List[torch.Tensor] = field(default_factory=list)
    steps_left: int = 1 << 60
    unquant_kv: Dict[int, torch.Tensor] = field(default_factory=dict)
    spec: Dict[int, tuple] = field(default_factory=dict)
    row_expanded: bool = False
    slot_guard: Dict[int, int] = field(default_factory=dict)
    slot_room: Dict[int, tuple] = field(default_factory=dict)


SpecResult = collections.namedtuple("SpecResult", "logits accepted tokens")


@dataclass
class LookupState:
    history: torch.Tensor
    hist_lens: torch.Tensor
    drafts: torch.Tensor
    match: torch.Tensor
    k: int
    max_ngram: int
    min_ngram: int


@dataclass
class SamplerState:
    temperature: torch.Tensor
    top_k: torch.Tensor
    top_p: torch.Tensor
    seeds: torch.Tensor
    draws: torch.Tensor
    logprobs: torch.Tensor
    u: torch.Tensor
    row_logprobs: Optional[torch.Tensor] = None
    row_u: Optional[torch.Tensor] = None
    row_bufs: Optional[Dict[int, tuple]] = None
    repetition_penalty: Optional[torch.Tensor] = None
    presence_penalty: Optional[torch.Tensor] = None
    seen: Optional[torch.Tensor] = None
    bias_ids: Optional[torch.Tensor] = None
    bias_vals: Optional[torch.Tensor] = None
    bias_cnt: Optional[torch.Tensor] = None
    bias_bits: Optional[torch.Tensor] = None
    top_n: int = 0
    top_ids: Optional[torch.Tensor] = None
    top_logprobs: Optional[torch.Tensor] = None
    row_top_ids: Optional[torch.Tensor] = None
    row_top_logprobs: Optional[torch.Tensor] = None
    row_top_bufs: Optional[Dict[int, tuple]] = None
    fsm: Optional[tuple] = None
    fsm_state: Optional[torch.Tensor] = None
    fsm_used: Optional[list] = None
    row_states: Optional[torch.Tensor] = None
    row_state_bufs: Optional[Dict[int, torch.Tensor]] = None

    def opts(self):
        kw = {}
        if self.bias_ids is not None:
            kw["bias"] = (self.bias_ids, self.bias_vals, self.bias_cnt, self.bias_bits)
        if self.top_n:
            kw.update(top_n=self.top_n, top_ids=self.top_ids, top_logprobs=self.top_logprobs)
        if self.fsm is not None:
            kw.update(fsm=self.fsm, fsm_state=self.fsm_state)
        return kw


@dataclass
class StopState:
    stop_ids: torch.Tensor
    stop_seqs: torch.Tensor
    seq_lens: torch.Tensor
    max_new: torch.Tensor
    gen_lens: torch.Tensor
    tail: torch.Tensor
    last_token: torch.Tensor
    finished: torch.Tensor
    emit_lens: torch.Tensor
    live: torch.Tensor

    def advance(self, new_tokens, ctx, accepted=None, next_tokens=None):
        ops.stop_advance(self.stop_ids, self.stop_seqs, self.seq_lens, self.max_new, self.gen_lens, self.tail, self.last_token, self.finished,
                         new_tokens, accepted=accepted, next_tokens=next_tokens, tokens=ctx.tokens, positions=ctx.positions,
                         placement=ctx.placement, valid_lens=ctx.valid_lens, emit_lens=self.emit_lens, live=self.live)


class _PromptRows:
    labels_dev = ks_rows = vs_rows = len_bufs_dev = plan = k_tab = v_tab = ks_tab = vs_tab = kv = kv_off = None
    last_rows = tasks_dev = ends_dev = None

    @classmethod
    def of(cls, model, ctx, tasks, prompts, pos0s, q8_history=False, labels=None):
# ... 58 lines not shown
        r.placement, r.len_q = r.pos.view(total, 1), 1
        r.buf_lens = ctx.buf_lens.index_select(0, rows_dev)
        r.k_rows, r.v_rows = ctx.k_addrs.index_select(1, rows_dev), ctx.v_addrs.index_select(1, rows_dev)
        if ctx.kv_quant:
            r.ks_rows, r.vs_rows = ctx.ks_addrs.index_select(1, rows_dev), ctx.vs_addrs.index_select(1, rows_dev)
        if q8_history:
            r.route, r.att_pos0s, r.len_bufs = "q8", pos0s, [ctx.max_len_buf] * n
            r.k_tab, r.v_tab = ctx.k_addrs.index_select(1, r.tasks_dev), ctx.v_addrs.index_select(1, r.tasks_dev)
            r.ks_tab, r.vs_tab = ctx.ks_addrs.index_select(1, r.tasks_dev), ctx.vs_addrs.index_select(1, r.tasks_dev)
        elif ctx.kv_quant:
            r.route, r.att_pos0s, r.len_bufs, r.len_bufs_dev = "own", [0] * n, lens, lens_dev
            r.kv_off = idx[2 * n + total:]
        else:
            r.route, r.att_pos0s, r.len_bufs = "cache", pos0s, [ctx.max_len_buf] * n
            r.k_tab, r.v_tab = ctx.k_addrs.index_select(1, r.tasks_dev), ctx.v_addrs.index_select(1, r.tasks_dev)
            r.len_bufs_dev = ctx.buf_lens.index_select(0, r.tasks_dev)
        if c.dim_head == 128:
            r.plan = ops.prefill_varlen_plan(lens, r.att_pos0s, r.len_bufs, dev)
        return r

    def att_tables(self, li, k3, v3):
        if self.route == "own":
            return self.kv_off + k3.data_ptr(), self.kv_off + v3.data_ptr()
        return self.k_tab[li], self.v_tab[li]


@dataclass(frozen=True)
class _DecodeRoute:
    qkv: str
    norm: Optional[str]
    attn: str
    out: str
    skip_attn: bool
    skip_proj: bool
    workspace: torch.Tensor
    scale: float
    merge_plan: Optional[tuple]
    la: Optional[tuple]
    stats: Optional[torch.Tensor]
    hook: object


class LLaMA:
    moe = False

    def __init__(self, cfg: ModelConfig, quant: QuantConfig, device="cuda:0", tp=None):
        if cfg.scale_depth > 0 and quant.quant_type != 0:
            raise ops.ZLError("scale_depth (MiniCPM residual scaling) is only wired into the unquantised layer stack")
        if quant.quant_type != 0 and cfg.torch_dtype != torch.float16:
            raise ops.ZLError("the W4A16 / int8 routes are fp16 (q_gemm_k_major.cu:989 asserts half)")
        self.cfg, self.quant, self.device = cfg, quant, torch.device(device)
        layer_cls = {0: DenseEncoderLayer, 2: Int8EncoderLayer}.get(quant.quant_type, EncoderLayer)
        self.tp = tp if tp is not None and tp.size > 1 else None
        self.full_cfg = cfg
        self.moe = any(cfg.is_moe_layer(i) for i in range(cfg.num_layers))
        if self.moe:
            if self.tp:
                raise ops.ZLError("MoE models: tensor parallelism is not supported")
            if layer_cls is not EncoderLayer:
                raise ops.ZLError("MoE models: GPTQ W4A16 checkpoints only")
            self.layers = [MoEEncoderLayer(cfg, quant, i) if cfg.is_moe_layer(i) else EncoderLayer(cfg, quant, i)
                           for i in range(cfg.num_layers)]
        elif self.tp:
            if layer_cls is not EncoderLayer:
                raise ops.ZLError("tensor parallelism is wired into the W4A16 layer stack only")
            t = self.tp.size
            kv_part = None
            if (cfg.num_kv_heads < t and t % cfg.num_kv_heads == 0 and int(os.environ.get("ATTN_KV_REP_TP", "0")) > 0):
                kv_part = (self.tp.rank // (t // cfg.num_kv_heads), cfg.num_kv_heads)
            if cfg.num_heads % t or (kv_part is None and cfg.num_kv_heads % t) or cfg.dim_ff % t or cfg.vocab_size % t:
                raise ops.ZLError("heads, kv heads, dim_ff and vocab_size must be divisible by the TP degree "
                                  "(fewer kv heads than ranks: ATTN_KV_REP_TP=1)")
            import dataclasses
            cfg = dataclasses.replace(cfg, num_heads=cfg.num_heads // t, num_kv_heads=1 if kv_part else cfg.num_kv_heads // t,
                                      dim_ff=cfg.dim_ff // t)
            self.cfg = cfg
            self.layers = [EncoderLayer(cfg, quant, i, self.tp) for i in range(cfg.num_layers)]
            for l in self.layers:
                l.kv_part = kv_part
        else:
            self.layers = [layer_cls(cfg, quant, i) for i in range(cfg.num_layers)]
        self.token_embedding = self.output_layernorm = self.lm_head = None
        self._bufs = {}

    def load_state_dict(self, state_dict: Dict[str, torch.Tensor], hf_names=True):
        sd = {hf_name_to_internal(k) if hf_names else k: v for k, v in state_dict.items()}
        dev = self.device
        dt = self.cfg.torch_dtype
        self.token_embedding = _dev_t(sd["llama.token_embedding.weight"], dev).to(dt).contiguous()
        self.output_layernorm = _dev_t(sd["llama.output_layernorm.weight"], dev).to(dt).contiguous()
        self.lm_head = self.token_embedding if self.cfg.tie_lm_head else _dev_t(sd["llama.lm_head.weight"], dev).to(dt).contiguous()
        if self.tp:
            v = self.cfg.vocab_size // self.tp.size
            self.lm_head = self.lm_head[self.tp.rank * v:(self.tp.rank + 1) * v].contiguous()
        for i, layer in enumerate(self.layers):
            layer.load_state_dict(sd, f"llama.layers.{i}", dev)
            layer.q_norm = layer.k_norm = None
            if self.cfg.qk_norm:
                layer.q_norm, layer.k_norm = (self._qk_norm_weight(sd[f"llama.layers.{i}.attn.{n}_norm.weight"], n)
                                              for n in ("q", "k"))
        return self

    def _qk_norm_weight(self, w, which):
        c, fc = self.cfg, self.full_cfg
        t = _dev_t(w, self.device).to(c.torch_dtype).reshape(-1)
        if c.qk_norm == "head":
            if t.numel() != c.dim_head:
                raise ops.ZLError("q_norm / k_norm weight must have dim_head elements")
            return t.contiguous()
        full = fc.num_heads if which == "q" else fc.num_kv_heads
        loc = c.num_heads if which == "q" else c.num_kv_heads
        if t.numel() != full * c.dim_head:
            raise ops.ZLError("q_norm / k_norm weight must have heads * dim_head elements")
        if self.tp:
            kv_part = getattr(self.layers[0], "kv_part", None)
            first = kv_part[0] if (which == "k" and kv_part) else self.tp.rank * loc
            t = t.view(full, c.dim_head)[first:first + loc]
        return t.contiguous()

    def apply_qk_norm(self, layer, qkv):
        c = self.cfg
        if not c.qk_norm:
            return
        hd, kvd = c.num_heads * c.dim_head, c.num_kv_heads * c.dim_head
        mode = 0 if c.qk_norm == "head" else 1
        ops.head_norm(qkv[:, :hd], layer.q_norm, c.num_heads, c.dim_head, c.eps, mode, out=qkv[:, :hd])
        ops.head_norm(qkv[:, hd:hd + kvd], layer.k_norm, c.num_kv_heads, c.dim_head, c.eps, mode, out=qkv[:, hd:hd + kvd])

    def init_random(self, seed=0):
        gen = torch.Generator(device=self.device).manual_seed(seed)
        c, dev = self.cfg, self.device
        dt = c.torch_dtype
        self.token_embedding = (torch.randn(c.vocab_size, c.dim_model, device=dev, generator=gen) * 0.5).to(dt)
        self.output_layernorm = torch.ones(c.dim_model, dtype=dt, device=dev)
        vloc = c.vocab_size // self.tp.size if self.tp else c.vocab_size
        self.lm_head = self.token_embedding if (c.tie_lm_head and not self.tp) else (torch.randn(vloc, c.dim_model, device=dev, generator=gen) * 0.02).to(dt)
        for layer in self.layers:
            layer.init_random(dev, gen)
            layer.q_norm = layer.k_norm = None
            if c.qk_norm:
                nq, nk = (c.dim_head, c.dim_head) if c.qk_norm == "head" else (c.num_heads * c.dim_head, c.num_kv_heads * c.dim_head)
                layer.q_norm = (1.0 + 0.1 * torch.randn(nq, device=dev, generator=gen)).to(dt)
                layer.k_norm = (1.0 + 0.1 * torch.randn(nk, device=dev, generator=gen)).to(dt)
        return self

    def init_synthetic(self, seed=0, sink=None):
        c, dev, q = self.cfg, self.device, self.quant
        if self.tp or not all(isinstance(l, EncoderLayer) for l in self.layers) or q.act_order or q.awq:
            raise ops.ZLError("init_synthetic: the plain GPTQ layer stack")
        gen = torch.Generator(device=dev).manual_seed(seed)
        g = q.group_size
        i64 = dict(dtype=torch.int64, device=dev, generator=gen)

        def pack8(nib, dim):
            word = torch.zeros_like(nib.select(dim, 0).unsqueeze(dim).expand(*[s // 8 if i == dim else s for i, s in enumerate(nib.shape)])).contiguous()
            for j in range(8):
                word |= (nib[j::8] if dim == 0 else nib[:, j::8]) << (4 * j)
            return torch.where(word >= 2 ** 31, word - 2 ** 32, word).to(torch.int32)

        def lin(sd, name, din, dout):
            sd[name + ".qweight"] = pack8(torch.randint(0, 16, (din, dout), **i64), 0)
            sd[name + ".qzeros"] = pack8(torch.randint(0, 15, (din // g, dout), **i64), 1)
            sd[name + ".scales"] = (torch.randn(din // g, dout, device=dev, generator=gen).abs() * ((0.5 / math.sqrt(din)) / 4) + 1e-4).to(torch.float16)
        hd, kvd = c.num_heads * c.dim_head, c.num_kv_heads * c.dim_head
        dt = c.torch_dtype
        for i, layer in enumerate(self.layers):
# ... 58 lines not shown
                kv_quant=True, kv_scales=kv_scales,
                ks_addrs=torch.tensor([[t[l, 0].data_ptr() for t in kv_scales] for l in range(c.num_layers)], dtype=torch.int64, device=dev),
                vs_addrs=torch.tensor([[t[l, 1].data_ptr() for t in kv_scales] for l in range(c.num_layers)], dtype=torch.int64, device=dev))
        k_addrs = torch.tensor([[t[l, 0].data_ptr() for t in kv] for l in range(c.num_layers)], dtype=torch.int64, device=dev)
        v_addrs = torch.tensor([[t[l, 1].data_ptr() for t in kv] for l in range(c.num_layers)], dtype=torch.int64, device=dev)
        i32 = dict(dtype=torch.int32, device=dev)
        return DynBatchContext(
            steps_left=len_buf - start_pos,
            tokens=torch.zeros(batch, **i32), positions=torch.full((batch,), start_pos, **i32),
            placement=torch.full((batch,), start_pos, **i32), buf_lens=torch.full((batch,), len_buf, **i32),
            valid_lens=torch.full((batch,), start_pos + 1, **i32), k_addrs=k_addrs, v_addrs=v_addrs,
            max_len_buf=len_buf, kv=kv, **quant_kw)

    def _buffers(self, b):
        if b not in self._bufs:
            c, dev = self.cfg, self.device
            f16 = dict(dtype=c.torch_dtype, device=dev)
            hd, kvd = c.num_heads * c.dim_head, c.num_kv_heads * c.dim_head
            self._bufs[b] = dict(
                hidden=torch.empty(b, c.dim_model, **f16), qkv=torch.empty(b, hd + 2 * kvd, **f16),
                q=torch.empty(b, hd, **f16), attn=torch.empty(b, hd, **f16), act=torch.empty(b, c.dim_ff, **f16),
                logits=torch.empty(b, c.vocab_size, **f16))
        return self._bufs[b]

    def _decode_route(self, ctx: DynBatchContext, b, gemv_only, skip_gemv, attend_rows, workspace=None) -> _DecodeRoute:
        c = self.cfg
        if (attend_rows is not None or self.moe) and (gemv_only or skip_gemv):
            raise ops.ZLError("gemv_only / skip_gemv: " + ("not with an attention hook" if attend_rows is not None else "dense models only"))
        if ctx.steps_left <= 0 and not torch.cuda.is_current_stream_capturing():
            raise ops.ZLError("decode step past the end of the KV buffers (placement >= len_buf): grow the buffers first "
                              "(the reference asserts pos_buf < len_buf, ragged_buffer_kernel.cu:194-222)")
        if workspace is None:
            workspace = self._bufs.setdefault(("ws", b, ctx.max_len_buf),
                                              ops.decode_attn_workspace(b, 1, c.num_heads, c.dim_head, ctx.max_len_buf, self.device))
        env, first = os.environ.get, self.layers[0]
        mfma_attn = c.dim_head == 128 and c.num_heads // c.num_kv_heads <= 16 and env("ZL_ATTN_MFMA", "1") != "0"
        fuse_rope = mfma_attn and not ctx.kv_quant and not c.qk_norm and env("ZL_FUSE_QKV_ROPE", "1") != "0"
        qkv, norm = "plain", None
        if (fuse_rope and all(isinstance(l, EncoderLayer) and l.unfused is None and l.qkv.perm is None
                              and isinstance(l.qkv.weight, ops.W4MWeight) for l in self.layers)
                and ops.w4_qkv_rope_scatter_ok(b, c.dim_model, c.dim_head, norm=b <= max(8, _fused_norm_rows(first.qkv.weight)))):
            qkv = "w4"
        elif fuse_rope and b <= 32 and c.dim_head % 32 == 0 and all(isinstance(l, Int8EncoderLayer) and l._stream(b) for l in self.layers):
            qkv = "w8"
        merge_plan = None
        if qkv == "w4" and not self.tp and attend_rows is None and env("ZL_ATTN_MERGE", "1") != "0" and all(l.attn_out.perm is None for l in self.layers):
            merge_plan = ops.attn_merge_plan(b, c.num_heads, c.num_kv_heads, c.dim_head, ctx.max_len_buf, first.attn_out.weight, c.torch_dtype)
        la, la_mode = None, env("ZL_ATTN_LA", _ATTN_LA_DEFAULT)
        if mfma_attn and not ctx.kv_quant and attend_rows is None and (la_mode == "1" or (la_mode == "auto" and merge_plan is None)):
            la_split = int(env("ZL_ATTN_LA_SPLIT", "0") or 0)
            eff = la_split or ops.decode_attn_la_split_len(b, c.num_kv_heads, ctx.max_len_buf)
            if (ctx.max_len_buf + eff - 1) // eff <= 64:
                key = ("la_ws", b, 1 << max(10, (ctx.max_len_buf - 1).bit_length()))
                if key not in self._bufs:
                    self._bufs[key] = ops.decode_attn_la_workspace(b, c.num_heads, c.num_kv_heads, key[2], self.device)
                la = (self._bufs[key], la_split, env("ZL_ATTN_LA_HALF", "0") == "1" and c.torch_dtype == torch.float16)
                merge_plan = None
        stats = None
        if (qkv == "w4" and (la is not None or attend_rows is not None) and not self.tp and not self.moe
                and env("ZL_ROW_SS", "1") != "0" and int(env("ZL_ROW_SS_MIN_M", "8")) <= b <= 32 and c.dim_model % 1024 == 0
                and all(l.attn_out.perm is None and l.w_out.perm is None and l.w_in_gated.perm is None for l in self.layers)
                and ops.w4_row_ss_routes(b, [first.attn_out.weight, first.w_out.weight],
                                         [(first.qkv.weight, True), (first.w_in_gated.weight, False)], self.device)):
            stats = self._bufs.get(("row_ss", b))
            if stats is None:
                stats = self._bufs[("row_ss", b)] = torch.empty((2, b, c.dim_model // 16), dtype=torch.float32, device=self.device)
        fuse_o_ff = (merge_plan is not None and merge_plan[2] and not self.moe and env("ZL_FUSE_O_GATEUP", "0") == "1" and ops.experimental_build()
                     and all(l.w_in_gated.perm is None and isinstance(l.w_in_gated.weight, ops.W4MWeight) for l in self.layers))
        if gemv_only and qkv == "plain":
            raise ops.ZLError("gemv_only: the fused W4 decode route only")
        if skip_gemv and qkv == "w4" and la is None and merge_plan is None:
            raise ops.ZLError("skip_gemv: the fused W4 decode route with the merging attn_out projection only")
        if qkv == "w4":
            norm = "row_ss" if stats is not None else "fused" if b <= max(8, _fused_norm_rows(first.qkv.weight)) else "launch"
        if ctx.kv_quant or attend_rows is not None:
            attn = "quant" if ctx.kv_quant else "hook"
        elif la is not None or merge_plan is not None:
            attn = "la" if la is not None else "splits"
        else:
            attn = "mqa" if qkv != "plain" or mfma_attn or ctx.row_expanded else "valu_fused"
        return _DecodeRoute(qkv, norm, attn, "merge_gate_up" if fuse_o_ff else "merge" if merge_plan is not None else "linear", skip_attn=gemv_only and qkv == "w4" and not skip_gemv, skip_proj=skip_gemv and qkv == "w4",
                            workspace=workspace, scale=1.0 / math.sqrt(c.dim_head), merge_plan=merge_plan, la=la, stats=stats, hook=attend_rows)

    def encode(self, ctx: DynBatchContext, workspace=None, argmax_ws=None, gemv_only=False, skip_gemv=False, attend_rows=None):
        c = self.cfg
        b = ctx.tokens.numel()
        r = self._decode_route(ctx, b, gemv_only, skip_gemv, attend_rows, workspace)
        bufs = self._buffers(b)
        rs = c.rope_scaling
        kind = rs.get("rope_type", rs.get("type")) if rs else None
        if gemv_only:
            hidden = bufs["hidden"]
            cos, sin = self._rope_tables(ctx.positions)
        elif kind in (None, "default", "llama3") and c.dim_head <= 256 and self.token_embedding.shape[0] == c.vocab_size:
            l3 = None if kind != "llama3" else (rs["factor"], rs["low_freq_factor"], rs["high_freq_factor"], rs["original_max_position_embeddings"])
            hidden, cos, sin = ops.embedding_rope(ctx.tokens, self.token_embedding, c.scale_emb, ctx.positions, c.dim_head, c.rope_theta, True, l3)
        else:
            hidden = ops.embedding(ctx.tokens, self.token_embedding, c.scale_emb)
            cos, sin = self._rope_tables(ctx.positions)
        if r.out == "merge_gate_up":
            ops.engine_epoch_advance(self.device)
        trace = getattr(self, "trace_hidden", None)
        for li, layer in enumerate(self.layers):
            if trace is not None and not torch.cuda.is_current_stream_capturing():
                trace.append(hidden.clone())
            if not r.skip_proj:
                self._decode_qkv(r, ctx, bufs, li, layer, hidden, cos, sin)
            if not r.skip_attn:
                self._decode_attend(r, ctx, bufs, li, cos, sin)
            if not r.skip_proj:
                self._decode_out_ff(r, ctx, bufs, li, layer, hidden)
        if gemv_only:
            return None
        self.last_hidden = hidden
        return self._logits(hidden, bufs["logits"], argmax_ws)

    def _decode_qkv(self, r, ctx, bufs, li, layer, hidden, cos, sin):
        c = self.cfg
        slots, heads = (ctx.placement, ctx.buf_lens, ctx.k_addrs[li], ctx.v_addrs[li]), (c.num_heads, c.num_kv_heads, c.dim_head)
        if r.qkv == "w4":
            if r.norm == "row_ss" and li == 0:
                ops.row_ss(hidden, out=r.stats[0])
            own = r.norm != "launch"
            ops.w4_qkv_rope_scatter(hidden if own else ops.rmsnorm(hidden, layer.ln_attn, c.eps), layer.qkv.weight, cos, sin, *slots,
                                    *heads, bias=layer.qkv.bias, norm_weight=layer.ln_attn if own else None, norm_eps=c.eps,
                                    q_out=bufs["q"], row_ss=r.stats[0] if r.norm == "row_ss" else None)
        elif r.qkv == "w8":
            _, xq, sx = ops.layernorm_quant(hidden, layer.ln_attn, c.eps)
            ops.w8a8_qkv_rope_scatter(xq, sx, layer.qkv.stream_weight(), cos, sin, *slots, *heads, q_out=bufs["q"])
        else:
            layer.project_qkv(hidden, c.eps, out=bufs["qkv"])
            self.apply_qk_norm(layer, bufs["qkv"])
            if r.attn == "quant":
                ops.rope_quant_scatter_decode(cos, sin, bufs["qkv"], *slots, ctx.ks_addrs[li], ctx.vs_addrs[li], *heads, q_out=bufs["q"])
            elif r.attn != "valu_fused":
                ops.rope_scatter_decode(cos, sin, bufs["qkv"], *slots, *heads, q_out=bufs["q"])

    def _decode_attend(self, r, ctx, bufs, li, cos, sin):
        c = self.cfg
        k, v, shape = ctx.k_addrs[li], ctx.v_addrs[li], (bufs["q"].shape[0], 1, c.num_heads, c.dim_head)
        if r.attn == "hook":
            r.hook(li, bufs["q"], bufs["attn"], r.workspace)
        elif r.attn == "la":
            ops.decode_attention_la(bufs["q"].view(shape), ctx.buf_lens, k, v, ctx.valid_lens, r.scale, ctx.max_len_buf, c.num_kv_heads,
                                    r.la[0], out=bufs["attn"].view(shape), split_len=r.la[1], half=r.la[2])
        elif r.attn == "splits":
            ops.decode_attention_splits(bufs["q"].view(shape[0], c.num_heads, c.dim_head), ctx.buf_lens, k, v, ctx.valid_lens, r.scale,
                                        ctx.max_len_buf, c.num_kv_heads, r.workspace)
        elif r.attn == "mqa":
            ops.multi_query_attention_rag_buffer(bufs["q"].view(shape), ctx.buf_lens, k, v, None, r.scale, ctx.max_len_buf, c.num_kv_heads,
                                                 valid_lens=ctx.valid_lens, out=bufs["attn"].view(shape), workspace=r.workspace)
        elif r.attn == "quant":
            ops.multi_query_attention_rag_buffer_quant(bufs["q"].view(shape), ctx.buf_lens, k, v, ctx.ks_addrs[li], ctx.vs_addrs[li], None,
                                                       r.scale, ctx.max_len_buf, c.num_kv_heads, valid_lens=ctx.valid_lens,
                                                       out=bufs["attn"].view(shape), workspace=r.workspace)
        else:
            ops.decode_attention_fused(cos, sin, bufs["qkv"], ctx.placement, ctx.buf_lens, ctx.valid_lens, k, v, c.num_heads, c.num_kv_heads,
                                       c.dim_head, r.scale, ctx.max_len_buf, out=bufs["attn"], workspace=r.workspace)

    def _decode_out_ff(self, r, ctx, bufs, li, layer, hidden):
        if r.norm == "row_ss":
            layer.attn_out.forward(bufs["attn"], residual=hidden, out=hidden, epilogue=ops.EPI_RESIDUAL, row_ss_out=r.stats[1])
            ops.w4_linear(hidden, layer.w_in_gated.weight, bias=layer.w_in_gated.bias, out=bufs["act"], norm_weight=layer.ln_ff,
                          norm_eps=self.cfg.eps, epilogue=ops.EPI_SILU_MUL, row_ss=r.stats[1])
            layer.w_out.forward(bufs["act"], residual=hidden, out=hidden, epilogue=ops.EPI_RESIDUAL, row_ss_out=r.stats[0])
            return
        if r.out == "linear":
            layer.attn_out_add(bufs["attn"], hidden)
        elif r.out == "merge_gate_up" and ops.w4_attn_out_gate_up(r.workspace, ctx.buf_lens, ctx.valid_lens, r.merge_plan, bufs["q"].shape[0],
                                                                   layer.attn_out.weight, hidden, layer.w_in_gated.weight, layer.ln_ff, self.cfg.eps,
                                                                   bufs["act"], li, bias_o=layer.attn_out.bias, bias_ff=layer.w_in_gated.bias):
            layer.w_out.forward(bufs["act"], residual=hidden, out=hidden, epilogue=ops.EPI_RESIDUAL)
            return
        else:
            ops.w4_attn_out_merge(r.workspace, ctx.buf_lens, ctx.valid_lens, r.merge_plan, bufs["q"].shape[0], layer.attn_out.weight,
                                  bias=layer.attn_out.bias, residual=hidden, out=hidden, epilogue=ops.EPI_RESIDUAL)
# ... 206 lines not shown
            raise
        index.commit(new)
        return logits, matched

    def score(self, ctx: DynBatchContext, tasks, prompts, pos0=None, labels=None, kv_history=None):
        if self.tp:
            raise ops.ZLError("score: tensor parallelism is not supported")
        tasks, pos0, q8_history = self._check_prompt_batch("score", ctx, tasks, prompts, pos0, kv_history)
        labels = ops.score_labels(prompts, labels)
        if any(l != ops.SCORE_IGNORE and not 0 <= l < self.cfg.vocab_size for l in labels):
            raise ops.ZLError("score: a label lies outside the vocabulary")
        r, hidden = self._prefill_rows(ctx, tasks, prompts, pos0, q8_history, labels)
        scored = self._score_rows(hidden, r.labels_dev, r.lens, r.last_rows)
        return scored._replace(logits=self._prompt_tail(ctx, r, hidden))

    def _score_rows(self, hidden, labels_dev, lens, last_rows=None):
        c = self.cfg
        ln_scale = (c.dim_model / c.dim_model_base) if c.dim_model_base > 0 else 1.0
        xn = ops.rmsnorm(hidden, self.output_layernorm, c.eps, ln_scale)
        if c.dim_model % 128 == 0:
            r = ops.lm_head_score(xn, self.lm_head, labels_dev)
        else:
            r = ops.lm_head_score_unfused(xn, self.lm_head, labels_dev)
        miss = ((r.greedy != labels_dev) & (labels_dev != ops.SCORE_IGNORE)).float()
        cu = [0]
        for s in lens:
            cu.append(cu[-1] + s)
        if last_rows is None:
            sums, matches = r.logprob.sum().view(1), (miss.sum() == 0).view(1)
        else:
            run = torch.stack([r.logprob.double(), miss.double()]).cumsum(1).index_select(1, last_rows)
            d = torch.diff(run, dim=1, prepend=run.new_zeros(2, 1))
            sums, matches = d[0].float(), d[1] == 0
        return ScoreResult(r.logprob, r.lse, r.greedy, r.greedy_logit, cu, sums, matches, None)

    def _prefill_rows(self, ctx: DynBatchContext, tasks, prompts, pos0s, q8_history=False, labels=None):
        c = self.cfg
        r = _PromptRows.of(self, ctx, tasks, prompts, pos0s, q8_history, labels)
        total = r.cu[-1]
        hidden = ops.embedding(r.tokens, self.token_embedding, c.scale_emb)
        cos, sin = self._rope_tables(r.pos)
        for li, layer in enumerate(self.layers):
            qkv = layer.project_qkv(hidden, c.eps)
            self.apply_qk_norm(layer, qkv)
            q, k, v = ops.rope_qk_cache(cos, sin, qkv, c.num_heads, c.num_kv_heads, c.dim_head, True)
            att = self._prompt_scatter_attend(r, li, q.view(total, c.num_heads, c.dim_head),
                                              k.view(total, c.num_kv_heads, c.dim_head), v.view(total, c.num_kv_heads, c.dim_head))
            layer.attn_out_add(att.view(total, -1), hidden)
            layer.ff_add(hidden, c.eps)
        return r, hidden

    def _prompt_scatter_attend(self, r, li, q3, k3, v3):
        c = self.cfg
        h, hkv, d = c.num_heads, c.num_kv_heads, c.dim_head
        scale = 1.0 / math.sqrt(d)
        k4, v4 = k3.view(*r.placement.shape, hkv, d), v3.view(*r.placement.shape, hkv, d)
        if r.ks_rows is None:
            ops.copy_to_rag_buffer2(r.placement, r.buf_lens, k4, v4, r.k_rows[li], r.v_rows[li])
        else:
            ops.quant_copy_to_rag_buffer(r.pos, r.buf_lens, k3, v3, r.k_rows[li], r.v_rows[li], r.ks_rows[li], r.vs_rows[li],
                                         len_q=r.len_q)
            if r.route == "temp":
                ops.copy_to_rag_buffer2(r.placement, r.len_bufs_dev, k4, v4, r.k_tab[li], r.v_tab[li])
        if d == 128:
            if r.route == "q8":
                return ops.prefill_attention_varlen_q8(q3, r.lens, r.att_pos0s, k3, v3, r.k_tab[li], r.v_tab[li], r.ks_tab[li],
                                                       r.vs_tab[li], r.len_bufs, hkv, scale, plan=r.plan)
            if r.plan is None:
                k_buf, v_buf = (k3, v3) if r.route == "own" else (r.kv[li, 0], r.kv[li, 1])
                return ops.prefill_attention(q3, k_buf, v_buf, r.att_pos0s[0], hkv, scale)
            return ops.prefill_attention_varlen(q3, r.lens, r.att_pos0s, *r.att_tables(li, k3, v3), r.plan.buf_lens, hkv, scale,
                                                plan=r.plan)
        k_tab, v_tab = r.att_tables(li, k3, v3)
        att = torch.empty_like(q3)
        for i, (s, p0) in enumerate(zip(r.lens, r.att_pos0s)):
            a = r.cu[i]
            mask, ws = self._prefill_mask(s, r.len_bufs[i], p0)
            ops.multi_query_attention_rag_buffer(q3[a:a + s].view(1, s, h, d), r.len_bufs_dev[i:i + 1], k_tab[i:i + 1],
                                                 v_tab[i:i + 1], mask, scale, r.len_bufs[i], hkv,
                                                 out=att[a:a + s].view(1, s, h, d), workspace=ws)
        return att

    def _prompt_tail(self, ctx, r, hidden):
        if r.tasks_dev is None:
            task, end = r.tasks[0], r.ends[0]
            logits = self._prompt_logits_and_pick(hidden[-1:], ctx.tokens[task:task + 1])
            ctx.positions[task] = end
            ctx.placement[task] = end
            ctx.valid_lens[task] = end + 1
        else:
            picks = torch.empty(len(r.tasks), dtype=torch.int32, device=self.device)
            logits = self._prompt_logits_and_pick(hidden.index_select(0, r.last_rows), picks)
            ctx.tokens.index_copy_(0, r.tasks_dev, picks)
            ctx.positions.index_copy_(0, r.tasks_dev, r.ends_dev)
            ctx.placement.index_copy_(0, r.tasks_dev, r.ends_dev)
            ctx.valid_lens.index_copy_(0, r.tasks_dev, r.ends_dev + 1)
        ctx.steps_left = min(ctx.steps_left, ctx.max_len_buf - max(r.ends))
        for t, end in zip(r.tasks, r.ends):
            ctx.slot_guard.pop(t, None)
            ctx.slot_room[t] = (ctx.max_len_buf - end, ctx.steps_left)
        return logits

    def _prompt_logits_and_pick(self, last_hidden, picks):
        n = last_hidden.shape[0]
        if self.tp:
            logits = self._logits(last_hidden)
            ops.argmax_advance(logits, tokens=picks)
            return logits
        key = ("argmax", n)
        if key not in self._bufs:
            self._bufs[key] = (ops.argmax_workspace(n, self.cfg.vocab_size, self.device),
                               torch.empty(n, dtype=torch.int64, device=self.device))
        ws = self._bufs[key][0]
        logits = self._logits(last_hidden, argmax_ws=ws)
        ops.greedy_advance(ws, n, self.cfg.vocab_size, tokens=picks)
        return logits

    def step_greedy(self, ctx: DynBatchContext, skip_gemv=False, stop: Optional[StopState] = None):
        b = ctx.tokens.numel()
        if stop is not None and stop.finished.numel() != b:
            raise ops.ZLError("step_greedy: the stop state belongs to another batch size")
        if b > 4 or self.tp:
            logits = self.encode(ctx)
            key = ("next", b)
            if key not in self._bufs:
                self._bufs[key] = torch.empty(b, dtype=torch.int64, device=self.device)
            nxt = self._bufs[key]
            ops.argmax_advance(logits, tokens=ctx.tokens, positions=ctx.positions, placement=ctx.placement, valid_lens=ctx.valid_lens,
                               next_tokens=nxt)
            if stop is not None:
                stop.advance(ctx.tokens.view(b, 1), ctx, next_tokens=nxt)
            ctx.steps_left -= 1
            return logits, nxt
        key = ("argmax", b)
        if key not in self._bufs:
            self._bufs[key] = (ops.argmax_workspace(b, self.cfg.vocab_size, self.device),
                               torch.empty(b, dtype=torch.int64, device=self.device))
        ws, nxt = self._bufs[key]
        logits = self.encode(ctx, argmax_ws=ws, skip_gemv=skip_gemv)
        ops.greedy_advance(ws, b, self.cfg.vocab_size, ctx.tokens, ctx.positions, ctx.placement, ctx.valid_lens, nxt)
        if stop is not None:
            stop.advance(ctx.tokens.view(b, 1), ctx, next_tokens=nxt)
        ctx.steps_left -= 1
        return logits, nxt

    @staticmethod
    def verify_route(b, len_q):
        return "causal" if b * len_q <= 4 else "rows"

    def verify(self, ctx: DynBatchContext, drafts: torch.Tensor, attn="auto", sampler: Optional[SamplerState] = None,
               stop: Optional[StopState] = None):
        c, dev = self.cfg, self.device
        if ctx.kv_quant:
            raise ops.ZLError("verify: not on the INT8 KV cache")
        if self.tp:
            raise ops.ZLError("verify: not under tensor parallelism")
        if c.dim_head != 128:
            raise ops.ZLError("verify: head size 128 only (the matrix-core decode attention)")
        if attn not in ("auto", "causal", "rows"):
            raise ops.ZLError("verify: attn is 'auto', 'causal' or 'rows'")
        b = ctx.tokens.numel()
        if not (torch.is_tensor(drafts) and drafts.dim() == 2 and drafts.shape[0] == b and drafts.shape[1] >= 1
                and drafts.dtype == torch.int32 and drafts.device == ctx.tokens.device and drafts.is_contiguous()):
            raise ops.ZLError("verify: drafts are (B, K) contiguous int32 on the context's device, K >= 1")
        if sampler is not None and sampler.temperature.numel() != b:
            raise ops.ZLError("verify: the sampler state belongs to another batch size")
        if stop is not None and stop.finished.numel() != b:
            raise ops.ZLError("verify: the stop state belongs to another batch size")
        len_q = drafts.shape[1] + 1
        m = b * len_q
        if attn == "auto":
            attn = self.verify_route(b, len_q)
        if len_q > 32 or m > 32:
            raise ops.ZLError("verify: at most 32 rows per step (B * (K + 1) <= 32)")
        capturing = torch.cuda.is_current_stream_capturing()
        if ctx.steps_left < len_q and not capturing:
            raise ops.ZLError("verify: the draft rows do not fit the KV buffers (steps_left < K + 1)")
        if len_q not in ctx.spec:
            if capturing:
                raise ops.ZLError("verify: run one eager call before capturing (it allocates the row-expanded view)")
            i32 = dict(dtype=torch.int32, device=dev)
            rows = DynBatchContext(
                tokens=torch.empty(m, **i32), positions=torch.empty(m, **i32), placement=torch.empty(m, **i32),
                valid_lens=torch.empty(m, **i32), buf_lens=torch.empty(m, **i32),
                k_addrs=torch.empty((c.num_layers, m), dtype=torch.int64, device=dev),
                v_addrs=torch.empty((c.num_layers, m), dtype=torch.int64, device=dev),
                max_len_buf=ctx.max_len_buf, kv=ctx.kv, row_expanded=True)
            ctx.spec[len_q] = (rows, torch.arange(len_q, **i32).view(1, len_q), torch.empty(b, **i32), torch.empty((b, len_q), **i32),
                               torch.arange(b, device=dev).view(b, 1).expand(b, len_q).reshape(m))
        rows, ar, accepted, out_tokens, task_of_row = ctx.spec[len_q]
        if sampler is not None:
            if sampler.row_bufs is None:
                sampler.row_bufs = {}
            if len_q not in sampler.row_bufs:
                if capturing:
                    raise ops.ZLError("verify: run one eager call with this sampler before capturing (it allocates the row results)")
                sampler.row_bufs[len_q] = tuple(torch.full((b, len_q), float("nan"), dtype=torch.float32, device=dev) for _ in range(2))
            sampler.row_logprobs, sampler.row_u = sampler.row_bufs[len_q]
            if sampler.fsm is not None:
                if sampler.row_state_bufs is None:
                    sampler.row_state_bufs = {}
                if len_q not in sampler.row_state_bufs:
                    if capturing:
                        raise ops.ZLError("verify: run one eager call with this sampler before capturing (it allocates the row results)")
                    sampler.row_state_bufs[len_q] = torch.full((b, len_q), -1, dtype=torch.int32, device=dev)
                sampler.row_states = sampler.row_state_bufs[len_q]
            if sampler.top_n:
                if sampler.row_top_bufs is None:
                    sampler.row_top_bufs = {}
                if len_q not in sampler.row_top_bufs:
                    if capturing:
                        raise ops.ZLError("verify: run one eager call with this sampler before capturing (it allocates the row results)")
                    sampler.row_top_bufs[len_q] = (torch.full((b, len_q, sampler.top_n), -1, dtype=torch.int32, device=dev),
                                                   torch.full((b, len_q, sampler.top_n), float("nan"), dtype=torch.float32, device=dev))
                sampler.row_top_ids, sampler.row_top_logprobs = sampler.row_top_bufs[len_q]
        torch.index_select(ctx.buf_lens, 0, task_of_row, out=rows.buf_lens)
        torch.index_select(ctx.k_addrs, 1, task_of_row, out=rows.k_addrs)
        torch.index_select(ctx.v_addrs, 1, task_of_row, out=rows.v_addrs)
        rows.max_len_buf, rows.kv = ctx.max_len_buf, ctx.kv
        tok = rows.tokens.view(b, len_q)
        tok[:, 0].copy_(ctx.tokens)
        tok[:, 1:].copy_(drafts.clamp(0, c.vocab_size - 1))
        torch.add(ctx.positions.view(b, 1), ar, out=rows.positions.view(b, len_q))
# ... 294 lines not shown
        i32 = dict(dtype=torch.int32, device=dev)
        tail = torch.full((b, ops.STOP_TAIL), -1, **i32)
        tail[:, ops.STOP_TAIL - 1].copy_(ctx.tokens)
        return StopState(stop_ids=sid, stop_seqs=ssq, seq_lens=sln, max_new=torch.tensor([int(v) for v in lim], **i32),
                         gen_lens=torch.zeros(b, **i32), tail=tail, last_token=ctx.tokens.clone(), finished=torch.zeros(b, **i32),
                         emit_lens=torch.zeros(b, **i32), live=torch.full((1,), b, **i32))

    def step_sample(self, ctx: DynBatchContext, state: SamplerState, stop: Optional[StopState] = None):
        b = ctx.tokens.numel()
        if state.temperature.numel() != b:
            raise ops.ZLError("step_sample: the state belongs to another batch size")
        if stop is not None and stop.finished.numel() != b:
            raise ops.ZLError("step_sample: the stop state belongs to another batch size")
        logits = self.encode(ctx)
        key = ("next", b)
        if key not in self._bufs:
            self._bufs[key] = torch.empty(b, dtype=torch.int64, device=self.device)
        nxt = self._bufs[key]
        ops.sample_advance(logits, state.temperature, state.top_k, state.top_p, seeds=state.seeds, draws=state.draws, tokens=ctx.tokens,
                           positions=ctx.positions, placement=ctx.placement, valid_lens=ctx.valid_lens, next_tokens=nxt,
                           logprobs=state.logprobs, u_out=state.u, rep_penalty=state.repetition_penalty, presence=state.presence_penalty,
                           seen=state.seen, **state.opts())
        if stop is not None:
            stop.advance(ctx.tokens.view(b, 1), ctx, next_tokens=nxt)
        ctx.steps_left -= 1
        return logits, nxt

    def generate_sample(self, ctx: DynBatchContext, state: SamplerState, max_new_tokens, stop: Optional[StopState] = None, poll=8):
        b, dev = ctx.tokens.numel(), ctx.tokens.device
        poll = int(poll)
        if stop is not None and poll < 1:
            raise ops.ZLError("generate_sample: poll >= 1")
        toks, lps, tis, tls = [], [], [], []
        for step in range(max(0, min(int(max_new_tokens), ctx.steps_left))):
            if stop is not None and step and step % poll == 0 and int(stop.live) == 0:
                break
            _, nxt = self.step_sample(ctx, state, stop)
            toks.append(nxt.clone())
            lps.append(state.logprobs.clone())
            if state.top_n:
                tis.append(state.top_ids.clone())
                tls.append(state.top_logprobs.clone())
        if not toks:
            out = (torch.empty((b, 0), dtype=torch.int64, device=dev), torch.empty((b, 0), dtype=torch.float32, device=dev))
            if state.top_n:
                out += ((torch.empty((b, 0, state.top_n), dtype=torch.int32, device=dev),
                         torch.empty((b, 0, state.top_n), dtype=torch.float32, device=dev)),)
            return out
        if state.top_n:
            return torch.stack(toks, dim=1), torch.stack(lps, dim=1), (torch.stack(tis, dim=1), torch.stack(tls, dim=1))
        return torch.stack(toks, dim=1), torch.stack(lps, dim=1)

    @staticmethod
    def slot_widths(sampler: Optional[SamplerState], stop: Optional[StopState], lookup: Optional[LookupState]):
        return ops.slot_widths(penalties=sampler is not None and sampler.seen is not None,
                               bias_ld=sampler.bias_ids.shape[1] if sampler is not None and sampler.bias_ids is not None else 0,
                               n_ids=stop.stop_ids.shape[1] if stop is not None else 0, n_seqs=stop.stop_seqs.shape[1] if stop is not None else 0,
                               seq_ld=stop.stop_seqs.shape[2] if stop is not None else 0,
                               hist_cap=lookup.history.shape[1] if lookup is not None else 0,
                               grammar=sampler is not None and sampler.fsm is not None)

    def _slot_states(self, what, ctx, sampler, stop, lookup):
        b = ctx.tokens.numel()
        if self.tp:
            raise ops.ZLError(f"{what}: tensor parallelism is not supported")
        if lookup is not None and ctx.kv_quant:
            raise ops.ZLError(f"{what}: lookup: not on the INT8 KV cache")
        if not isinstance(sampler, SamplerState) or sampler.temperature.numel() != b:
            raise ops.ZLError(f"{what}: the sampler state belongs to another batch size")
        if stop is not None and stop.finished.numel() != b:
            raise ops.ZLError(f"{what}: the stop state belongs to another batch size")
        if lookup is not None and (lookup.history.shape[0] != b or lookup.drafts.shape != (b, lookup.k)):
            raise ops.ZLError(f"{what}: the lookup state belongs to another batch size")
        return b

    def _slots_launch(self, ctx, blob, sampler, stop, lookup, parked_ok=None):
        b = ctx.tokens.numel()
        new = None
        if lookup is not None:
            key = ("draft_new", b)
            if key not in self._bufs:
                self._bufs[key] = torch.empty(b, dtype=torch.int32, device=self.device)
            new = self._bufs[key]
        ops.slots_admit(blob, ctx.tokens, ctx.positions, ctx.placement, ctx.valid_lens, sampler=sampler, stop=stop, lookup=lookup,
                        draft_new=new, parked_ok=parked_ok)
        if lookup is not None:
            ops.lookup_draft(lookup.history, lookup.hist_lens, lookup.k, lookup.max_ngram, lookup.min_ngram, new_tokens=new.view(b, 1),
                             drafts=lookup.drafts, match=lookup.match)

    def _steps_left_after_admission(self, ctx, before):
        left = {}
        for t in range(ctx.tokens.numel()):
            if t in ctx.slot_guard:
                ctx.slot_room.pop(t, None)
                continue
            room, at = ctx.slot_room.get(t, (before, before))
            left[t] = max(before, room - (at - before)) if at >= before else before
        ctx.steps_left = min(left.values()) if left else 1 << 60
        ctx.slot_room.update({t: (v, ctx.steps_left) for t, v in left.items()})

    def admit(self, ctx: DynBatchContext, slots, prompts, requests, sampler: SamplerState, stop: Optional[StopState] = None,
              lookup: Optional[LookupState] = None, cache=None, kv_history=None):
        b = self._slot_states("admit", ctx, sampler, stop, lookup)
        prompts = list(prompts)
        requests = [dict(rq or {}) for rq in requests]
        for j, rq in enumerate(requests if len(requests) == len(prompts) else []):
            if rq.get("grammar") is not None:
                pr = torch.as_tensor(prompts[j]).reshape(-1)
                g = rq["grammar"]
                if isinstance(g, bool) or not isinstance(g, (int, np.integer)):
                    raise ops.ZLError("admit: grammar is load_grammar's start state")
                if sampler.fsm is None or not 0 <= int(g) < sampler.fsm_used[0]:
                    raise ops.ZLError("admit: grammar names no loaded automaton of this sampler")
                if pr.numel() < 2:
                    raise ops.ZLError("admit: a request with a grammar needs a prompt of 2 tokens at least (the last one is re-fed)")
                prompts[j], rq["grammar"] = pr[:-1], (int(g), int(pr[-1]))
        slots, _, _ = self._check_prompt_batch("admit", ctx, slots, prompts, None, kv_history)
        if len(requests) != len(slots):
            raise ops.ZLError("admit: one request per slot")
        k = lookup.k if lookup is not None else 0
        entries, guards = [], {}
        for s, pr, rq in zip(slots, prompts, requests):
            n = int(pr.numel())
            if stop is not None:
                raw = rq.get("max_new_tokens", 0)
                if isinstance(raw, bool) or not isinstance(raw, (int, np.integer)) or not 0 <= int(raw) < 1 << 31:
                    raise ops.ZLError(f"admit: slot {s}: max_new_tokens is an integer >= 0 (0 = no limit)")
                lim = ops.slot_max_new(n, int(raw), ctx.max_len_buf, k)
                if lim < 1:
                    raise ops.ZLError(f"admit: prompt of slot {s} ({n} tokens) leaves no room for one generated token")
                rq["max_new_tokens"] = lim
                guards[s] = n + lim + k + 1
            if lookup is not None and rq.get("history") is None:
                rq["history"] = pr.reshape(-1)
            entries.append((s, rq))
        blob, _ = ops.slots_pack(entries, self.cfg.vocab_size, self.slot_widths(sampler, stop, lookup))
        before = ctx.steps_left
        if cache is None:
            out = self.prefill_batch(ctx, slots, prompts, kv_history=kv_history)
        else:
            out = self.prefill_cached(ctx, cache, slots, prompts, kv_history=kv_history)
        self._slots_launch(ctx, blob, sampler, stop, lookup)
        if guards:
            ctx.slot_guard.update(guards)
            self._steps_left_after_admission(ctx, before)
        return out

    def park(self, ctx: DynBatchContext, slots, sampler: SamplerState, stop: StopState, lookup: Optional[LookupState] = None, finished=None):
        b = self._slot_states("park", ctx, sampler, stop, lookup)
        slots = [int(s) for s in slots]
        if stop is None:
            raise ops.ZLError("park: needs the stop state (only a finished slot is parked)")
        if not slots or len(set(slots)) != len(slots) or any(s < 0 or s >= b for s in slots):
            raise ops.ZLError("park: slots must be distinct indices of the batch")
        done = [] if finished is None else [int(v) for v in (finished.tolist() if hasattr(finished, "tolist") else finished)]
        if len(done) != b or any(done[s] == 0 for s in slots):
            raise ops.ZLError("park: only a slot known to be finished is parked (finished = the host copy of stop.finished)")
        blob, _ = ops.slots_pack([(s, None) for s in slots], self.cfg.vocab_size, self.slot_widths(sampler, stop, lookup))
        self._slots_launch(ctx, blob, sampler, stop, lookup, parked_ok=set(slots))
        before = ctx.steps_left
        ctx.slot_guard.update({s: 0 for s in slots})
        self._steps_left_after_admission(ctx, before)

    def advance(self, ctx: DynBatchContext, next_tokens: torch.Tensor):
        ctx.tokens.copy_(next_tokens.to(torch.int32))
        ctx.positions.add_(1)
# ... 7 lines not shown
```

### zhilight_amd/ops.py

```python
import collections
import ctypes as C
import os
import math

import numpy as np
import torch

from . import _lib
from ._lib import W4Layout, W4Opts, ZLError, check, lib

F16, BF16 = 0, 1
EPI_BIAS, EPI_ADD_C, EPI_RESIDUAL, EPI_SILU_MUL, EPI_SILU_MUL_F32 = 1, 2, 4, 8, 16


def _stream():
    return C.c_void_p(torch.cuda.current_stream().cuda_stream)


def _p(t):
    return C.c_void_p(0 if t is None else t.data_ptr())


def _i(v):
    return C.c_int64(int(v))
# ... 603 lines not shown
    if out is None:
        out = torch.empty((m, n), dtype=x.dtype, device=x.device)
    else:
        _chk_out(out, m, n, x.dtype, x.device, "gemm_nt_small_m")
    if argmax_ws is None:
        check(lib().zl_gemm_nt_small_m(_p(x2), _i(x2.stride(0)), _p(weight), _p(bias), _p(out), _i(m), _i(n), _i(k),
                                       _f(alpha), C.c_int(_dt(x)), _p(norm_weight), _f(norm_eps), _stream()),
              "gemm_nt_small_m")
    else:
        check(lib().zl_gemm_nt_small_m_argmax(_p(x2), _i(x2.stride(0)), _p(weight), _p(bias), _p(out), _i(m), _i(n),
                                              _i(k), _f(alpha), C.c_int(_dt(x)), _p(norm_weight), _f(norm_eps),
                                              _p(argmax_ws), _stream()), "gemm_nt_small_m_argmax")
    return out


def gemm_nt(x, weight, bias=None, alpha=1.0, out=None):
    _chk_cuda(x, weight, bias)
    x2 = x.reshape(-1, x.shape[-1])
    m, k = x2.shape
    n = weight.shape[0]
    if weight.shape[1] != k:
        raise ZLError("size K mismatch")
    if out is None:
        out = torch.empty((m, n), dtype=x.dtype, device=x.device)
    else:
        _chk_out(out, m, n, x.dtype, x.device, "gemm_nt")
    check(lib().zl_gemm_nt(_p(x2), _i(x2.stride(0)), _p(weight), _p(bias), _p(out), _i(m), _i(n), _i(k), _f(alpha),
                           C.c_int(_dt(x)), _stream()), "gemm_nt")
    return out


class DenseMWeight:

    def __init__(self, weight):
        _chk_cuda(weight)
        n, k = weight.shape
        nbytes = int(lib().zl_dense_m_bytes(_i(n), _i(k)))
        if nbytes < 0:
            check(nbytes, "dense_m_bytes")
        self.n, self.k, self.dtype = n, k, weight.dtype
        self.data = torch.empty(nbytes // 2, dtype=weight.dtype, device=weight.device)
        w = weight if weight.is_contiguous() else weight.contiguous()
        check(lib().zl_dense_pack_m(_p(w), _p(self.data), _i(n), _i(k), _stream()), "dense_pack_m")


def gemm_nt_packed(x, w, bias=None, alpha=1.0, out=None):
    _chk_cuda(x, bias)
    x2 = x.reshape(-1, x.shape[-1])
    m, k = x2.shape
    if k != w.k or x.dtype != w.dtype:
        raise ZLError("gemm_nt_packed: size K / dtype mismatch")
    if out is None:
        out = torch.empty((m, w.n), dtype=x.dtype, device=x.device)
    else:
        _chk_out(out, m, w.n, x.dtype, x.device, "gemm_nt_packed")
    check(lib().zl_gemm_nt_packed(_p(x2), _i(x2.stride(0)), _p(w.data), _p(bias), _p(out), _i(m), _i(w.n), _i(k), _f(alpha),
                                  C.c_int(_dt(x)), _stream()), "gemm_nt_packed")
    return out


def gemm_nt_f32(x, weight, alpha=1.0):
    _chk_cuda(x, weight)
    x2 = x.reshape(-1, x.shape[-1])
    m, k = x2.shape
    n = weight.shape[0]
    if weight.shape[1] != k or weight.dtype != x.dtype:
        raise ZLError("size K / dtype mismatch")
    out = torch.empty((m, n), dtype=torch.float32, device=x.device)
    check(lib().zl_gemm_nt_f32(_p(x2), _i(x2.stride(0)), _p(weight), _p(out), _i(m), _i(n), _i(k), _f(alpha), C.c_int(_dt(x)), _stream()), "gemm_nt_f32")
    return out


def argmax_workspace(m, n, device):
    nbytes = lib().zl_argmax_workspace_bytes(_i(m), _i(n))
    if nbytes < 0:
        check(int(nbytes), "argmax_workspace_bytes")
    return torch.empty(nbytes // 4, dtype=torch.float32, device=device)


def greedy_advance(argmax_ws, m, n, tokens=None, positions=None, placement=None, valid_lens=None, next_tokens=None):
    _chk_cuda(argmax_ws, tokens, positions, placement, valid_lens, next_tokens)
    check(lib().zl_greedy_advance(_p(argmax_ws), _i(m), _i(n), _p(tokens), _p(positions), _p(placement),
                                  _p(valid_lens), _p(next_tokens), _stream()), "greedy_advance")
    return next_tokens


def argmax_advance(logits, tokens=None, positions=None, placement=None, valid_lens=None, next_tokens=None):
    _chk_cuda(tokens, positions, placement, valid_lens, next_tokens)
    if not (logits.is_cuda and logits.dim() == 2 and logits.stride(1) == 1 and logits.stride(0) >= logits.shape[1]):
        raise ZLError("argmax_advance: (rows, n) CUDA logits with unit column stride")
    rows, n = logits.shape
    code = {torch.float16: 2, torch.bfloat16: 6, torch.float32: 1}[logits.dtype]
    check(lib().zl_argmax_advance(_p(logits), C.c_int(code), _i(rows), _i(n), _i(logits.stride(0)), _p(tokens), _p(positions), _p(placement),
                                  _p(valid_lens), _p(next_tokens), _stream()), "argmax_advance")
    return next_tokens if next_tokens is not None else tokens


def spec_accept(logits, drafts, tokens=None, positions=None, placement=None, valid_lens=None, accepted=None, out_tokens=None):
    if not (torch.is_tensor(logits) and torch.is_tensor(drafts)):
        raise ZLError("spec_accept: logits and drafts are tensors")
    if logits.dim() != 2 or logits.stride(1) != 1 or logits.stride(0) < logits.shape[1] or logits.shape[1] < 1:
        raise ZLError("spec_accept: (B * len_q, n) logits with unit column stride")
    if logits.dtype not in (torch.float16, torch.bfloat16, torch.float32):
        raise ZLError(f"spec_accept: unsupported logits dtype {logits.dtype}")
    if drafts.dim() != 2 or drafts.shape[1] < 1 or drafts.dtype != torch.int32 or not drafts.is_contiguous():
        raise ZLError("spec_accept: drafts are (B, K) contiguous int32, K >= 1")
    b, len_q = drafts.shape[0], drafts.shape[1] + 1
    if b < 1 or logits.shape[0] != b * len_q:
        raise ZLError("spec_accept: one logit row per task and draft position: B * (K + 1) rows")
    if not logits.is_cuda or drafts.device != logits.device:
        raise ZLError("spec_accept: CUDA logits, drafts on the logits' device")
    for t, what in ((tokens, "tokens"), (positions, "positions"), (placement, "placement"), (valid_lens, "valid_lens"), (accepted, "accepted")):
        if t is not None and (t.dtype != torch.int32 or t.numel() != b or not t.is_contiguous() or t.device != logits.device):
            raise ZLError(f"spec_accept: {what}: contiguous int32 of length B on the logits' device")
    if accepted is None:
        accepted = torch.empty(b, dtype=torch.int32, device=logits.device)
    if out_tokens is None:
        out_tokens = torch.empty((b, len_q), dtype=torch.int32, device=logits.device)
    elif out_tokens.dtype != torch.int32 or out_tokens.numel() != b * len_q or not out_tokens.is_contiguous() or out_tokens.device != logits.device:
        raise ZLError("spec_accept: out_tokens: contiguous int32 (B, K + 1) on the logits' device")
    code = {torch.float16: 2, torch.bfloat16: 6, torch.float32: 1}[logits.dtype]
    check(lib().zl_spec_accept(_p(logits), C.c_int(code), _i(b), _i(len_q), _i(logits.shape[1]), _i(logits.stride(0)), _p(drafts), _p(tokens),
                               _p(positions), _p(placement), _p(valid_lens), _p(accepted), _p(out_tokens), _stream()), "spec_accept")
    return accepted, out_tokens.view(b, len_q)


def lookup_draft(history, hist_lens, k, max_ngram=3, min_ngram=1, new_tokens=None, drafts=None, match=None):
    if not (torch.is_tensor(history) and torch.is_tensor(hist_lens)):
        raise ZLError("lookup_draft: history and hist_lens are tensors")
    if history.dim() != 2 or history.dtype != torch.int32 or not history.is_contiguous() or history.shape[0] < 1 or history.shape[1] < 2:
        raise ZLError("lookup_draft: history is (B, cap) contiguous int32, cap >= 2")
    b, cap = history.shape
    if cap >= 1 << 31:
        raise ZLError("lookup_draft: a history row holds fewer than 2^31 ids")
    if hist_lens.dtype != torch.int32 or hist_lens.dim() != 1 or hist_lens.numel() != b or not hist_lens.is_contiguous():
        raise ZLError("lookup_draft: hist_lens is (B) contiguous int32")
    k, max_ngram, min_ngram = int(k), int(max_ngram), int(min_ngram)
    if not 1 <= k <= 31:
        raise ZLError("lookup_draft: 1 <= k <= 31 (a verify step has at most 32 rows per task)")
    if not 1 <= min_ngram <= max_ngram <= 16:
        raise ZLError("lookup_draft: 1 <= min_ngram <= max_ngram <= 16")
    n_new = 0
    if new_tokens is not None:
        if not (torch.is_tensor(new_tokens) and new_tokens.dim() == 2 and new_tokens.shape[0] == b and 1 <= new_tokens.shape[1] <= 32
                and new_tokens.dtype == torch.int32 and new_tokens.is_contiguous()):
            raise ZLError("lookup_draft: new_tokens is (B, n_new) contiguous int32, 1 <= n_new <= 32")
        n_new = new_tokens.shape[1]
    if drafts is not None and not (torch.is_tensor(drafts) and drafts.dtype == torch.int32 and drafts.numel() == b * k
                                   and drafts.is_contiguous()):
        raise ZLError("lookup_draft: drafts: contiguous int32 (B, k)")
    if match is not None and not (torch.is_tensor(match) and match.dtype == torch.int32 and match.numel() == b * 2 and match.is_contiguous()):
        raise ZLError("lookup_draft: match: contiguous int32 (B, 2)")
    if not history.is_cuda or any(t is not None and t.device != history.device for t in (hist_lens, new_tokens, drafts, match)):
        raise ZLError("lookup_draft: CUDA history, every other tensor on the history's device")
    if drafts is None:
        drafts = torch.empty((b, k), dtype=torch.int32, device=history.device)
    if match is None:
        match = torch.empty((b, 2), dtype=torch.int32, device=history.device)
    check(lib().zl_lookup_draft(_p(history), _i(cap), _p(hist_lens), _p(new_tokens), _i(n_new), _i(b), _i(k), C.c_int(max_ngram),
                                C.c_int(min_ngram), _p(drafts), _p(match), _stream()), "lookup_draft")
    return drafts.view(b, k), match.view(b, 2)


STOP_IDS_MAX = 16
STOP_SEQS_MAX = 8
STOP_SEQ_LEN_MAX = 16
# ... 2058 lines not shown
```

Before: 647.3 tokens/s.

## Fuse greedy token pick with next-step embedding and rope table generation

The greedy advance kernel now also gathers the embedding row for the chosen token and writes the rope cos/sin rows for the next position. The next decode step reuses these staged buffers, validated by an epoch and tensor-version mark, instead of launching the separate embedding+rope kernel. The split-merge path of the w4 GEMM also gains a KS template so few-split cases load per-lane stats and reduce them with DPP/swizzle instead of unrolled loads over 16 records. The staging adds state tracking that could go stale if the invalidation checks miss a case.

After: 644.8 tokens/s. Within noise of the previous version (-0.4%).

```diff
diff --git a/include/zhilight_amd.h b/include/zhilight_amd.h
--- a/include/zhilight_amd.h
+++ b/include/zhilight_amd.h
@@ -142,6 +142,10 @@
                               const uint16_t* norm_weight, float norm_eps, void* argmax_ws, zl_stream_t s);
 int zl_greedy_advance(const void* argmax_ws, int64_t m, int64_t n, int32_t* tokens, int32_t* positions,
                       int32_t* placement, int32_t* valid_lens, int64_t* next_tokens, zl_stream_t s);
+int zl_greedy_advance_embed(const void* argmax_ws, int64_t m, int64_t n, int32_t* tokens, int32_t* positions, int32_t* placement,
+                            int32_t* valid_lens, int64_t* next_tokens, const uint16_t* weight, uint16_t* hidden, int64_t dim, float scale,
+                            int dtype, float* cosv, float* sinv, int64_t d, float base, int neox, int llama3, float factor,
+                            float low_freq_factor, float high_freq_factor, float old_context_len, zl_stream_t s);
 
 int64_t zl_lm_head_score_ws_bytes(int64_t m, int64_t n);
 int zl_lm_head_score(const uint16_t* x, int64_t ldx, const uint16_t* w , const int32_t* labels, int32_t ignore_index,
diff --git a/zhilight_amd/_lib.py b/zhilight_amd/_lib.py
--- a/zhilight_amd/_lib.py
+++ b/zhilight_amd/_lib.py
@@ -19,7 +19,7 @@
     "zl_awq_un_shuffle", "zl_awq_shuffle",
     "zl_w4_layout", "zl_w4_pack", "zl_w4_dequant", "zl_w4a16_gemm",
     "zl_w4m_layout", "zl_w4m_pack", "zl_w4m_unpack", "zl_w4a16_gemm_mfma", "zl_w4a16_gemm_tiled", "zl_w4a16_scratch_bytes", "zl_w4a16_gemm_mfma_ex", "zl_w4a16_gemm_tiled_ex",
-    "zl_gemm_nt_small_m", "zl_gemm_nt", "zl_gemm_nt_f32", "zl_argmax_workspace_bytes", "zl_gemm_nt_small_m_argmax", "zl_greedy_advance",
+    "zl_gemm_nt_small_m", "zl_gemm_nt", "zl_gemm_nt_f32", "zl_argmax_workspace_bytes", "zl_gemm_nt_small_m_argmax", "zl_greedy_advance", "zl_greedy_advance_embed",
     "zl_lm_head_score_ws_bytes", "zl_lm_head_score", "zl_lm_head_score_ex",
     "zl_rmsnorm",
     "zl_w4a16_moe_up", "zl_w4a16_moe_down", "zl_moe_grouped_bm", "zl_moe_grouped_tiles", "zl_w4a16_gemm_grouped", "zl_w4a16_gemm_pairs", "zl_rope_cos_sin", "zl_rope_cos_sin_llama3", "zl_rope_cos_sin_dynamic", "zl_rope_cos_sin_yarn", "zl_head_norm", "zl_rotary_embedding_qk", "zl_rope_qk_cache", "zl_rope_rotate", "zl_mask_valid_lens",
diff --git a/zhilight_amd/csrc/dense_gemv.hip b/zhilight_amd/csrc/dense_gemv.hip
--- a/zhilight_amd/csrc/dense_gemv.hip
+++ b/zhilight_amd/csrc/dense_gemv.hip
@@ -1,4 +1,5 @@
 #include "zl_common.h"
+#include "zl_embed_rope.h"
 #include "zl_stage.h"
 
 namespace {
@@ -134,12 +135,7 @@
     return v > bv || (v == bv && i < bi);
 }
 
-__global__ __launch_bounds__(256) void k_greedy_advance(const float2* ws, int total_waves, int32_t* tokens,
-                                                        int32_t* positions, int32_t* placement, int32_t* valid_lens,
-                                                        int64_t* next_out) {
-    __shared__ float sv[256];
-    __shared__ int si[256];
-    const int b = blockIdx.x;
+__device__ __forceinline__ int greedy_pick(const float2* ws, int total_waves, int b, float* sv, int* si) {
     float bv = -INFINITY;
     int bi = 0x7fffffff;
     for (int w0 = threadIdx.x; w0 < total_waves; w0 += 4 * 256) {
@@ -172,14 +168,51 @@
         }
         __syncthreads();
     }
+    return si[0] == 0x7fffffff ? 0 : si[0];
+}
+
+__global__ __launch_bounds__(256) void k_greedy_advance(const float2* ws, int total_waves, int32_t* tokens,
+                                                        int32_t* positions, int32_t* placement, int32_t* valid_lens,
+                                                        int64_t* next_out) {
+    __shared__ float sv[256];
+    __shared__ int si[256];
+    const int b = blockIdx.x;
+    const int tok = greedy_pick(ws, total_waves, b, sv, si);
     if (threadIdx.x == 0) {
-        const int tok = si[0] == 0x7fffffff ? 0 : si[0];
         if (tokens) tokens[b] = tok;
         if (next_out) next_out[b] = tok;
         if (positions) positions[b] += 1;
         if (placement) placement[b] += 1;
         if (valid_lens) valid_lens[b] += 1;
     }
+}
+
+struct GreedyEmbed {
+    const uint16_t* w;
+    uint16_t* hidden;
+    float *cosv, *sinv;
+    int dim, vocab, d, neox, llama3;
+    float scale, base, factor, low_ff, high_ff, old_ctx;
+};
+template <int DT>
+__global__ __launch_bounds__(256) void k_greedy_advance_embed(const float2* ws, int total_waves, int32_t* tokens, int32_t* positions,
+                                                              int32_t* placement, int32_t* valid_lens, int64_t* next_out, const GreedyEmbed e) {
+    __shared__ float sv[256];
+    __shared__ int si[256];
+    const int b = blockIdx.x;
+    const int next_pos = positions[b] + 1;
+    float inv_freq = 0.f;
+    if ((int)threadIdx.x < e.d) inv_freq = zl_rope_inv_freq(threadIdx.x, e.d, e.base, e.neox, e.llama3, e.factor, e.low_ff, e.high_ff, e.old_ctx);
+    const int tok = greedy_pick(ws, total_waves, b, sv, si);
+    if (threadIdx.x == 0) {
+        tokens[b] = tok;
+        if (next_out) next_out[b] = tok;
+        positions[b] = next_pos;
+        if (placement) placement[b] += 1;
+        if (valid_lens) valid_lens[b] += 1;
+    }
+    zl_embedding_row_id<DT>(b, tok, e.w, e.hidden, e.dim, 0, e.vocab, e.scale);
+    if ((int)threadIdx.x < e.d) zl_rope_cos_sin_store(b, next_pos, inv_freq, e.cosv, e.sinv, e.d);
 }
 
 template <int DT, int MT>
@@ -296,3 +329,25 @@
                        reinterpret_cast<const float2*>(argmax_ws), tw, tokens, positions, placement, valid_lens, next_tokens);
     return zl_launch_status();
 }
+
+extern "C" int zl_greedy_advance_embed(const void* argmax_ws, int64_t m, int64_t n, int32_t* tokens, int32_t* positions, int32_t* placement,
+                                       int32_t* valid_lens, int64_t* next_tokens, const uint16_t* weight, uint16_t* hidden, int64_t dim,
+                                       float scale, int dtype, float* cosv, float* sinv, int64_t d, float base, int neox, int llama3,
+                                       float factor, float low_freq_factor, float high_freq_factor, float old_context_len, zl_stream_t s) {
+    ZL_CHECK_ARG(argmax_ws && m > 0 && n > 0 && tokens && positions && weight && hidden && cosv && sinv && dim > 0 && d > 0, ZL_EINVAL);
+    ZL_CHECK_ARG(d <= 256 && d % 2 == 0 && n < ((int64_t)1 << 31) && dim < ((int64_t)1 << 31), ZL_ESHAPE);
+    ZL_CHECK_ARG(dtype == ZL_F16 || dtype == ZL_BF16, ZL_EDTYPE);
+    int rpw, gx;
+    const int tw = dense_waves(n, &rpw, &gx);
+    GreedyEmbed e;
+    e.w = weight; e.hidden = hidden; e.cosv = cosv; e.sinv = sinv;
+    e.dim = (int)dim; e.vocab = (int)n; e.d = (int)d; e.neox = neox; e.llama3 = llama3;
+    e.scale = scale; e.base = base; e.factor = factor; e.low_ff = low_freq_factor; e.high_ff = high_freq_factor; e.old_ctx = old_context_len;
+    if (dtype == ZL_F16)
+        hipLaunchKernelGGL(k_greedy_advance_embed<ZL_F16>, dim3((unsigned)m), dim3(256), 0, (hipStream_t)s,
+                           reinterpret_cast<const float2*>(argmax_ws), tw, tokens, positions, placement, valid_lens, next_tokens, e);
+    else
+        hipLaunchKernelGGL(k_greedy_advance_embed<ZL_BF16>, dim3((unsigned)m), dim3(256), 0, (hipStream_t)s,
+                           reinterpret_cast<const float2*>(argmax_ws), tw, tokens, positions, placement, valid_lens, next_tokens, e);
+    return zl_launch_status();
+}
diff --git a/zhilight_amd/csrc/misc_ops.hip b/zhilight_amd/csrc/misc_ops.hip
--- a/zhilight_amd/csrc/misc_ops.hip
+++ b/zhilight_amd/csrc/misc_ops.hip
@@ -1,5 +1,6 @@
 #include <mutex>
 #include "zl_common.h"
+#include "zl_embed_rope.h"
 
 namespace {
 
@@ -49,33 +50,6 @@
     }
 }
 
-__device__ __forceinline__ int half_dim_index(int col, int half_dim, int neox) {
-    return neox ? (col < half_dim ? col : col - half_dim) : col / 2;
-}
-
-__device__ __forceinline__ void rope_cos_sin_row(int row, const int32_t* __restrict__ pos, float* __restrict__ cosv, float* __restrict__ sinv,
-                                                 int d, float base, int neox, int llama3, float factor, float low_ff, float high_ff,
-                                                 float old_ctx) {
-    const int col = threadIdx.x;
-    if (col >= d) return;
-    const int i = half_dim_index(col, d / 2, neox);
-    float inv_freq = (float)pow((double)base, (double)(-(float)(i * 2) / (float)d));
-    if (llama3) {
-        const float low_wl = old_ctx / low_ff, high_wl = old_ctx / high_ff;
-        const float pi = 3.141592653589793f;
-        const float wavelen = 2.f * pi / inv_freq;
-        if (wavelen < high_wl) {
-        } else if (wavelen > low_wl) {
-            inv_freq = inv_freq / factor;
-        } else {
-            const float smooth = (old_ctx / wavelen - low_ff) / (high_ff - low_ff);
-            inv_freq = __builtin_fmaf(smooth, inv_freq, (1.f - smooth) * inv_freq / factor);
-        }
-    }
-    const float freq = (float)pos[row] * inv_freq;
-    cosv[(size_t)row * d + col] = cosf(freq);
-    sinv[(size_t)row * d + col] = sinf(freq);
-}
 __global__ void k_rope_cos_sin(const int32_t* __restrict__ pos, float* __restrict__ cosv, float* __restrict__ sinv,
                                int d, float base, int neox, int llama3, float factor, float low_ff, float high_ff,
                                float old_ctx) {
@@ -361,33 +335,6 @@
 }
 
 template <int DT>
-__device__ __forceinline__ void embedding_row(int row, const int32_t* __restrict__ ids, const uint16_t* __restrict__ w,
-                                              uint16_t* __restrict__ out, int dim, int begin, int end, float scale) {
-    int id = ids[row];
-    const bool in_range = id >= begin && id < end;
-    id -= begin;
-    const uint16_t* src = w + (size_t)(in_range ? id : 0) * dim;
-    uint16_t* dst = out + (size_t)row * dim;
-    if ((dim & 7) == 0 && ((((uintptr_t)w) | ((uintptr_t)out)) & 15) == 0) {
-        const int chunks = dim >> 3;
-        for (int c0 = threadIdx.x; c0 < chunks; c0 += 2 * blockDim.x) {
-            const int c1 = c0 + blockDim.x;
-            uint4 v0 = *reinterpret_cast<const uint4*>(src + (size_t)c0 * 8), v1 = make_uint4(0, 0, 0, 0);
-            if (c1 < chunks) v1 = *reinterpret_cast<const uint4*>(src + (size_t)c1 * 8);
-            auto conv = [&](uint32_t u) {
-                const uint16_t lo = in_range ? ZT<DT>::from_f32(ZT<DT>::to_f32((uint16_t)(u & 0xffffu)) * scale) : ZT<DT>::from_f32(0.f);
-                const uint16_t hi = in_range ? ZT<DT>::from_f32(ZT<DT>::to_f32((uint16_t)(u >> 16)) * scale) : ZT<DT>::from_f32(0.f);
-                return (uint32_t)lo | ((uint32_t)hi << 16);
-            };
-            *reinterpret_cast<uint4*>(dst + (size_t)c0 * 8) = make_uint4(conv(v0.x), conv(v0.y), conv(v0.z), conv(v0.w));
-            if (c1 < chunks) *reinterpret_cast<uint4*>(dst + (size_t)c1 * 8) = make_uint4(conv(v1.x), conv(v1.y), conv(v1.z), conv(v1.w));
-        }
-        return;
-    }
-    for (int i = threadIdx.x; i < dim; i += blockDim.x)
-        dst[i] = in_range ? ZT<DT>::from_f32(ZT<DT>::to_f32(src[i]) * scale) : ZT<DT>::from_f32(0.f);
-}
-template <int DT>
 __global__ void k_embedding(const int32_t* __restrict__ ids, const uint16_t* __restrict__ w, uint16_t* __restrict__ out,
                             int dim, int begin, int end, float scale) {
     embedding_row<DT>(blockIdx.x, ids, w, out, dim, begin, end, scale);
diff --git a/zhilight_amd/csrc/w4_i8p.hip b/zhilight_amd/csrc/w4_i8p.hip
--- a/zhilight_amd/csrc/w4_i8p.hip
+++ b/zhilight_amd/csrc/w4_i8p.hip
@@ -1,3 +1,4 @@
+#include <utility>
 #include "zl_common.h"
 #include "w4_i8p_common.h"
 
@@ -26,10 +27,31 @@
 #define ZL_IPROBE(slot) do {} while (0)
 #endif
 
-template <int R, bool LONGK, bool ROPE, bool NORM, bool MERGE = false>
+template <int... U, class F>
+__device__ __forceinline__ void zl_static_for(std::integer_sequence<int, U...>, F&& f) {
+    (f(std::integral_constant<int, U>{}), ...);
+}
+template <int N>
+__device__ __forceinline__ float zl_row16_lane(float v) {
+    return __builtin_bit_cast(float, __builtin_amdgcn_ds_swizzle(__builtin_bit_cast(int, v), 0x10 | (N << 5)));
+}
+template <int CTRL>
+__device__ __forceinline__ float zl_dpp_mov(float v) {
+    return __builtin_bit_cast(float, __builtin_amdgcn_update_dpp(0, __builtin_bit_cast(int, v), CTRL, 0xf, 0xf, true));
+}
+__device__ __forceinline__ float zl_row16_max(float v) {
+    v = fmaxf(v, zl_dpp_mov<0xB1>(v));
+    v = fmaxf(v, zl_dpp_mov<0x4E>(v));
+    v = fmaxf(v, zl_dpp_mov<0x141>(v));
+    v = fmaxf(v, zl_dpp_mov<0x140>(v));
+    return v;
+}
+
+template <int R, bool LONGK, bool ROPE, bool NORM, bool MERGE = false, int KS = 16>
 __global__ __launch_bounds__(kT, 2) void k_w4a16_i8p(const I8Params p) {
     static_assert(!ROPE || R == 2, "fused rotary: a tile and its partner tile");
     static_assert(!MERGE || (!LONGK && !ROPE && !NORM), "split merge: one column block, plain prologue");
+    static_assert(KS >= 1 && KS <= 16 && (MERGE || KS == 16), "split merge: up to 16 records, one per lane of a head's 16");
     constexpr int XD = R >= ZL_I8P_RING ? 1 : (ZL_I8P_RING / R > 0 ? ZL_I8P_RING / R : 1);
     constexpr int D = R * XD;
     constexpr int NS = LONGK ? 8 : 4;
@@ -89,32 +111,34 @@
         xr[s] = make_uint4(0, 0, 0, 0);
         if constexpr (MERGE) {
             if (row < M) {
-                constexpr int kS = 16;
+                constexpr int kS = KS;
                 const int head = g < groups ? g : 0;
                 const uint32_t n_rec = (uint32_t)M * (uint32_t)groups * (uint32_t)p.mg_max_splits;
                 const __amdgpu_buffer_rsrc_t rpart = __builtin_amdgcn_make_buffer_rsrc(const_cast<uint16_t*>(p.mg_part), 0, n_rec * 256u, 0x00020000);
                 const __amdgpu_buffer_rsrc_t rstat = __builtin_amdgcn_make_buffer_rsrc(const_cast<float*>(p.mg_stat), 0, n_rec * 8u, 0x00020000);
                 const uint32_t rec0 = ((uint32_t)row * (uint32_t)groups + (uint32_t)head) * (uint32_t)p.mg_max_splits;
-                const uint32_t po = rec0 * 256u + (uint32_t)uo * 16u, so = rec0 * 8u;
+                const uint32_t po = rec0 * 256u + (uint32_t)uo * 16u;
+                const uint32_t so = (rec0 + ((int)uo < p.mg_max_splits ? (uint32_t)uo : 0u)) * 8u;
+                const float2 st = __builtin_bit_cast(float2, __builtin_amdgcn_raw_buffer_load_b64(rstat, so, 0, 0));
                 uint4 pv[kS];
-                float2 st[kS];
 #pragma unroll
                 for (int u = 0; u < kS; ++u) {
                     const uint32_t uc = u < p.mg_max_splits ? (uint32_t)u : 0u;
                     pv[u] = __builtin_bit_cast(uint4, __builtin_amdgcn_raw_buffer_load_b128(rpart, po, uc * 256u, 0));
-                    st[u] = __builtin_bit_cast(float2, __builtin_amdgcn_raw_buffer_load_b64(rstat, so, uc * 8u, 0));
-                }
+                }
+                __builtin_amdgcn_fence(__ATOMIC_RELEASE, "wavefront");
                 if (s == 0) issue_early();
                 const int elen = min(p.buf_lens[row], p.mg_valid_lens[row]);
                 const int ns = min((elen + p.mg_split_len - 1) / p.mg_split_len, kS);
-                float mn = -1e20f;
-#pragma unroll
-                for (int u = 0; u < kS; ++u) mn = fmaxf(mn, u < ns ? st[u].x : -1e20f);
+                const float mn = fmaxf(-1e20f, zl_row16_max((int)uo < ns ? st.x : -1e20f));
+                const float f_own = st.y * __expf(st.x - mn);
+                float fs[kS];
+                zl_static_for(std::make_integer_sequence<int, kS>{}, [&](auto U) { fs[U.value] = zl_row16_lane<U.value>(f_own); });
                 float a[8] = {0.f, 0.f, 0.f, 0.f, 0.f, 0.f, 0.f, 0.f}, z = 0.f;
 #pragma unroll
                 for (int u = 0; u < kS; ++u) {
                     if (u < ns) {
-                        const float f = st[u].y * __expf(st[u].x - mn);
+                        const float f = fs[u];
                         const uint32_t w4[4] = {pv[u].x, pv[u].y, pv[u].z, pv[u].w};
 #pragma unroll
                         for (int e = 0; e < 4; ++e) {
@@ -383,17 +407,26 @@
     return kW * gw * 8 * 64 * (size_t)m + kW * gw * 64 + (size_t)r * kW * 64 * 4 + 4 * kW * 4;
 }
 
-template <int R, bool LONGK, bool ROPE, bool NORM, bool MERGE = false>
+template <int R, bool LONGK, bool ROPE, bool NORM, bool MERGE = false, int KS = 16>
 int launch_i8p_n(const I8Params& p, int grid, hipStream_t hs) {
     const size_t lds = i8p_lds_bytes(p.groups, p.m, R);
     if (lds > 160 * 1024) return ZL_ELIMIT;
     if (lds > 64 * 1024) {
-        hipError_t e = hipFuncSetAttribute(reinterpret_cast<const void*>(&k_w4a16_i8p<R, LONGK, ROPE, NORM, MERGE>),
+        hipError_t e = hipFuncSetAttribute(reinterpret_cast<const void*>(&k_w4a16_i8p<R, LONGK, ROPE, NORM, MERGE, KS>),
                                            hipFuncAttributeMaxDynamicSharedMemorySize, (int)lds);
         if (e != hipSuccess) return ZL_ELIMIT;
     }
-    hipLaunchKernelGGL((k_w4a16_i8p<R, LONGK, ROPE, NORM, MERGE>), dim3(grid), dim3(kT), lds, hs, p);
+    hipLaunchKernelGGL((k_w4a16_i8p<R, LONGK, ROPE, NORM, MERGE, KS>), dim3(grid), dim3(kT), lds, hs, p);
     return zl_launch_status();
+}
+template <int R>
+int launch_i8p_merge(const I8Params& p, int grid, hipStream_t hs) {
+    if constexpr (R <= 2) {
+        if (p.mg_max_splits <= 4) return launch_i8p_n<R, false, false, false, true, 4>(p, grid, hs);
+        if (p.mg_max_splits <= 8) return launch_i8p_n<R, false, false, false, true, 8>(p, grid, hs);
+        if (p.mg_max_splits <= 12) return launch_i8p_n<R, false, false, false, true, 12>(p, grid, hs);
+    }
+    return launch_i8p_n<R, false, false, false, true, 16>(p, grid, hs);
 }
 template <int R, bool ROPE>
 int launch_i8p(const I8Params& p, int grid, hipStream_t hs) {
@@ -443,7 +476,7 @@
     int r = (pb.tiles + cus - 1) / cus;
     if (r > 8) r = 8;
     const int grid = (pb.tiles + r - 1) / r;
-#define ZL_I8M(RR) case RR: return launch_i8p_n<RR, false, false, false, true>(p, grid, hs);
+#define ZL_I8M(RR) case RR: return launch_i8p_merge<RR>(p, grid, hs);
     switch (r) { ZL_I8M(1) ZL_I8M(2) ZL_I8M(3) ZL_I8M(4) ZL_I8M(5) ZL_I8M(6) ZL_I8M(7) ZL_I8M(8) }
 #undef ZL_I8M
     return ZL_EINVAL;
diff --git a/zhilight_amd/csrc/zl_embed_rope.h b/zhilight_amd/csrc/zl_embed_rope.h
--- /dev/null
+++ b/zhilight_amd/csrc/zl_embed_rope.h
@@ -0,0 +1,71 @@
+#pragma once
+#include "zl_common.h"
+
+template <int DT>
+__device__ __forceinline__ void zl_embedding_row_id(int row, int id, const uint16_t* __restrict__ w, uint16_t* __restrict__ out, int dim,
+                                                    int begin, int end, float scale) {
+    const bool in_range = id >= begin && id < end;
+    id -= begin;
+    const uint16_t* src = w + (size_t)(in_range ? id : 0) * dim;
+    uint16_t* dst = out + (size_t)row * dim;
+    if ((dim & 7) == 0 && ((((uintptr_t)w) | ((uintptr_t)out)) & 15) == 0) {
+        const int chunks = dim >> 3;
+        for (int c0 = threadIdx.x; c0 < chunks; c0 += 2 * blockDim.x) {
+            const int c1 = c0 + blockDim.x;
+            uint4 v0 = *reinterpret_cast<const uint4*>(src + (size_t)c0 * 8), v1 = make_uint4(0, 0, 0, 0);
+            if (c1 < chunks) v1 = *reinterpret_cast<const uint4*>(src + (size_t)c1 * 8);
+            auto conv = [&](uint32_t u) {
+                const uint16_t lo = in_range ? ZT<DT>::from_f32(ZT<DT>::to_f32((uint16_t)(u & 0xffffu)) * scale) : ZT<DT>::from_f32(0.f);
+                const uint16_t hi = in_range ? ZT<DT>::from_f32(ZT<DT>::to_f32((uint16_t)(u >> 16)) * scale) : ZT<DT>::from_f32(0.f);
+                return (uint32_t)lo | ((uint32_t)hi << 16);
+            };
+            *reinterpret_cast<uint4*>(dst + (size_t)c0 * 8) = make_uint4(conv(v0.x), conv(v0.y), conv(v0.z), conv(v0.w));
+            if (c1 < chunks) *reinterpret_cast<uint4*>(dst + (size_t)c1 * 8) = make_uint4(conv(v1.x), conv(v1.y), conv(v1.z), conv(v1.w));
+        }
+        return;
+    }
+    for (int i = threadIdx.x; i < dim; i += blockDim.x)
+        dst[i] = in_range ? ZT<DT>::from_f32(ZT<DT>::to_f32(src[i]) * scale) : ZT<DT>::from_f32(0.f);
+}
+template <int DT>
+__device__ __forceinline__ void embedding_row(int row, const int32_t* __restrict__ ids, const uint16_t* __restrict__ w,
+                                              uint16_t* __restrict__ out, int dim, int begin, int end, float scale) {
+    zl_embedding_row_id<DT>(row, ids[row], w, out, dim, begin, end, scale);
+}
+
+__device__ __forceinline__ int half_dim_index(int col, int half_dim, int neox) {
+    return neox ? (col < half_dim ? col : col - half_dim) : col / 2;
+}
+
+__device__ __forceinline__ float zl_rope_inv_freq(int col, int d, float base, int neox, int llama3, float factor, float low_ff, float high_ff,
+                                                  float old_ctx) {
+    const int i = half_dim_index(col, d / 2, neox);
+    float inv_freq = (float)pow((double)base, (double)(-(float)(i * 2) / (float)d));
+    if (llama3) {
+        const float low_wl = old_ctx / low_ff, high_wl = old_ctx / high_ff;
+        const float pi = 3.141592653589793f;
+        const float wavelen = 2.f * pi / inv_freq;
+        if (wavelen < high_wl) {
+        } else if (wavelen > low_wl) {
+            inv_freq = inv_freq / factor;
+        } else {
+            const float smooth = (old_ctx / wavelen - low_ff) / (high_ff - low_ff);
+            inv_freq = __builtin_fmaf(smooth, inv_freq, (1.f - smooth) * inv_freq / factor);
+        }
+    }
+    return inv_freq;
+}
+__device__ __forceinline__ void zl_rope_cos_sin_store(int row, int position, float inv_freq, float* __restrict__ cosv, float* __restrict__ sinv, int d) {
+    const int col = threadIdx.x;
+    const float freq = (float)position * inv_freq;
+    cosv[(size_t)row * d + col] = cosf(freq);
+    sinv[(size_t)row * d + col] = sinf(freq);
+}
+__device__ __forceinline__ void rope_cos_sin_row(int row, const int32_t* __restrict__ pos, float* __restrict__ cosv, float* __restrict__ sinv,
+                                                 int d, float base, int neox, int llama3, float factor, float low_ff, float high_ff,
+                                                 float old_ctx) {
+    const int col = threadIdx.x;
+    if (col >= d) return;
+    const float inv_freq = zl_rope_inv_freq(col, d, base, neox, llama3, factor, low_ff, high_ff, old_ctx);
+    zl_rope_cos_sin_store(row, pos[row], inv_freq, cosv, sinv, d);
+}
diff --git a/zhilight_amd/llama.py b/zhilight_amd/llama.py
--- a/zhilight_amd/llama.py
+++ b/zhilight_amd/llama.py
@@ -788,6 +788,8 @@
     row_expanded: bool = False
     slot_guard: Dict[int, int] = field(default_factory=dict)
     slot_room: Dict[int, tuple] = field(default_factory=dict)
+    staged_rows: Optional[tuple] = None
+    staged_at: Optional[tuple] = None
 
 
 SpecResult = collections.namedtuple("SpecResult", "logits accepted tokens")
@@ -1012,6 +1014,7 @@
             self.layers = [layer_cls(cfg, quant, i) for i in range(cfg.num_layers)]
         self.token_embedding = self.output_layernorm = self.lm_head = None
         self._bufs = {}
+        self._epoch = 0
 
     def load_state_dict(self, state_dict: Dict[str, torch.Tensor], hf_names=True):
         sd = {hf_name_to_internal(k) if hf_names else k: v for k, v in state_dict.items()}
@@ -1236,9 +1239,10 @@
         return _DecodeRoute(qkv, norm, attn, "merge_gate_up" if fuse_o_ff else "merge" if merge_plan is not None else "linear", skip_attn=gemv_only and qkv == "w4" and not skip_gemv, skip_proj=skip_gemv and qkv == "w4",
                             workspace=workspace, scale=1.0 / math.sqrt(c.dim_head), merge_plan=merge_plan, la=la, stats=stats, hook=attend_rows)
 
-    def encode(self, ctx: DynBatchContext, workspace=None, argmax_ws=None, gemv_only=False, skip_gemv=False, attend_rows=None):
+    def encode(self, ctx: DynBatchContext, workspace=None, argmax_ws=None, gemv_only=False, skip_gemv=False, attend_rows=None, staged=None):
         c = self.cfg
         b = ctx.tokens.numel()
+        self._epoch += 1
         r = self._decode_route(ctx, b, gemv_only, skip_gemv, attend_rows, workspace)
         bufs = self._buffers(b)
         rs = c.rope_scaling
@@ -1246,6 +1250,8 @@
         if gemv_only:
             hidden = bufs["hidden"]
             cos, sin = self._rope_tables(ctx.positions)
+        elif staged is not None:
+            hidden, cos, sin = staged
         elif kind in (None, "default", "llama3") and c.dim_head <= 256 and self.token_embedding.shape[0] == c.vocab_size:
             l3 = None if kind != "llama3" else (rs["factor"], rs["low_freq_factor"], rs["high_freq_factor"], rs["original_max_position_embeddings"])
             hidden, cos, sin = ops.embedding_rope(ctx.tokens, self.token_embedding, c.scale_emb, ctx.positions, c.dim_head, c.rope_theta, True, l3)
@@ -1618,6 +1624,7 @@
         return att
 
     def _prompt_tail(self, ctx, r, hidden):
+        self._epoch += 1
         if r.tasks_dev is None:
             task, end = r.tasks[0], r.ends[0]
             logits = self._prompt_logits_and_pick(hidden[-1:], ctx.tokens[task:task + 1])
@@ -1673,8 +1680,28 @@
             self._bufs[key] = (ops.argmax_workspace(b, self.cfg.vocab_size, self.device),
                                torch.empty(b, dtype=torch.int64, device=self.device))
         ws, nxt = self._bufs[key]
-        logits = self.encode(ctx, argmax_ws=ws, skip_gemv=skip_gemv)
-        ops.greedy_advance(ws, b, self.cfg.vocab_size, ctx.tokens, ctx.positions, ctx.placement, ctx.valid_lens, nxt)
+        c, rs = self.cfg, self.cfg.rope_scaling
+        kind = rs.get("rope_type", rs.get("type")) if rs else None
+        handoff = (stop is None and os.environ.get("ZL_STEP_HANDOFF", "1") != "0" and kind in (None, "default", "llama3") and c.dim_head <= 256
+                   and self.token_embedding.shape[0] == c.vocab_size and getattr(self, "trace_hidden", None) is None)
+
+        def mark():
+            return (id(self), self._epoch, ctx.tokens._version, ctx.positions._version, ctx.tokens.data_ptr(), ctx.positions.data_ptr())
+        staged = ctx.staged_rows if handoff and ctx.staged_rows is not None and ctx.staged_at == mark() else None
+        logits = self.encode(ctx, argmax_ws=ws, skip_gemv=skip_gemv, staged=staged)
+        if handoff:
+            if ctx.staged_rows is None:
+                f32 = dict(dtype=torch.float32, device=self.device)
+                ctx.staged_rows = (torch.empty(b, c.dim_model, dtype=c.torch_dtype, device=self.device),
+                                   torch.empty(b, c.dim_head, **f32), torch.empty(b, c.dim_head, **f32))
+            l3 = None if kind != "llama3" else (rs["factor"], rs["low_freq_factor"], rs["high_freq_factor"], rs["original_max_position_embeddings"])
+            ops.greedy_advance_embed(ws, b, c.vocab_size, ctx.tokens, ctx.positions, ctx.placement, ctx.valid_lens, nxt, self.token_embedding,
+                                     c.scale_emb, *ctx.staged_rows, c.rope_theta, True, l3)
+            ctx.staged_at = mark()
+            if staged is not None:
+                self.last_hidden = None
+        else:
+            ops.greedy_advance(ws, b, self.cfg.vocab_size, ctx.tokens, ctx.positions, ctx.placement, ctx.valid_lens, nxt)
         if stop is not None:
             stop.advance(ctx.tokens.view(b, 1), ctx, next_tokens=nxt)
         ctx.steps_left -= 1
@@ -2135,6 +2162,7 @@
             if key not in self._bufs:
                 self._bufs[key] = torch.empty(b, dtype=torch.int32, device=self.device)
             new = self._bufs[key]
+        self._epoch += 1
         ops.slots_admit(blob, ctx.tokens, ctx.positions, ctx.placement, ctx.valid_lens, sampler=sampler, stop=stop, lookup=lookup,
                         draft_new=new, parked_ok=parked_ok)
         if lookup is not None:
diff --git a/zhilight_amd/ops.py b/zhilight_amd/ops.py
--- a/zhilight_amd/ops.py
+++ b/zhilight_amd/ops.py
@@ -709,6 +709,21 @@
     _chk_cuda(argmax_ws, tokens, positions, placement, valid_lens, next_tokens)
     check(lib().zl_greedy_advance(_p(argmax_ws), _i(m), _i(n), _p(tokens), _p(positions), _p(placement),
                                   _p(valid_lens), _p(next_tokens), _stream()), "greedy_advance")
+    return next_tokens
+
+
+def greedy_advance_embed(argmax_ws, m, n, tokens, positions, placement, valid_lens, next_tokens, weight, scale, hidden, cos, sin, base,
+                         neox=True, llama3=None):
+    _chk_cuda(argmax_ws, tokens, positions, placement, valid_lens, next_tokens, weight, hidden, cos, sin)
+    if (weight.shape[0] != n or hidden.dtype != weight.dtype or tuple(hidden.shape) != (m, weight.shape[1]) or not hidden.is_contiguous()
+            or cos.dtype != torch.float32 or sin.dtype != torch.float32 or cos.shape != sin.shape or cos.shape[0] != m
+            or not cos.is_contiguous() or not sin.is_contiguous()):
+        raise ZLError("greedy_advance_embed: hidden (m, dim) of the embedding's type, cos / sin (m, dim_head) fp32, one weight row per id")
+    fac, low, high, old = llama3 if llama3 is not None else (1.0, 1.0, 1.0, 1.0)
+    check(lib().zl_greedy_advance_embed(_p(argmax_ws), _i(m), _i(n), _p(tokens), _p(positions), _p(placement), _p(valid_lens),
+                                        _p(next_tokens), _p(weight), _p(hidden), _i(weight.shape[1]), _f(scale), C.c_int(_dt(weight)),
+                                        _p(cos), _p(sin), _i(cos.shape[1]), _f(base), C.c_int(int(neox)), C.c_int(int(llama3 is not None)),
+                                        _f(fac), _f(low), _f(high), _f(old), _stream()), "greedy_advance_embed")
     return next_tokens
 
 
```
